# nkwangyh/CubemapSLAM

Hardware: AMD Instinct MI355X
Metric: frames/sec (extract+match+localBA) on Lafida cam0 (higher is better)
Workload: dtype u8 (extract/match), f64 (BA)

## Files before the change

cubemapslam_amd/api.py:

```python
import time
import ctypes as C
import os
import numpy as np

_HERE = os.path.dirname(os.path.abspath(__file__))
LIB_PATH = os.environ.get("CMS_HIP_LIB") or os.path.join(_HERE, "lib", "libcubemapslam_hip.so")


class CmsError(RuntimeError):
    pass


class Camera(C.Structure):
    _fields_ = [("c", C.c_double), ("d", C.c_double), ("e", C.c_double), ("u0", C.c_double), ("v0", C.c_double),
                ("invpol", C.c_double * 12), ("pol", C.c_double * 5), ("Iw", C.c_int), ("Ih", C.c_int),
                ("face", C.c_int), ("fov_deg", C.c_double)]


class OrbParams(C.Structure):
    _fields_ = [("nfeatures", C.c_int), ("scale_factor", C.c_float), ("nlevels", C.c_int),
                ("ini_th_fast", C.c_int), ("min_th_fast", C.c_int)]


class Geometry(C.Structure):
# ... 302 lines not shown
        f = lib().cms_stream_wait_extracted
        f.argtypes = [C.c_void_p, C.c_void_p]
        _chk(f(self.h, C.c_void_p(int(hip_stream))), "cms_stream_wait_extracted")

    def upload_wait(self):
        _chk(lib().cms_frames_upload_wait(self.h), "cms_frames_upload_wait")

    def process(self, B, from_fisheye=True):
        _chk(lib().cms_frames_process(self.h, B, 1 if from_fisheye else 0), "cms_frames_process")

    def sync(self):
        _chk(lib().cms_frames_sync(self.h), "cms_frames_sync")

    def fetch(self, b):
        cap = self.geom.kp_cap
        kps = np.zeros(cap, KP_DTYPE)
        desc = np.zeros((cap, 32), np.uint8)
        n = C.c_int()
        _chk(lib().cms_frames_fetch(self.h, b, _p(kps), _p(desc), cap, C.byref(n)), "cms_frames_fetch")
        return kps[:n.value].copy(), desc[:n.value].copy()

    def results_ptrs(self):
        a, b, c = C.c_void_p(), C.c_void_p(), C.c_void_p()
        _chk(lib().cms_frames_results(self.h, C.byref(a), C.byref(b), C.byref(c)), "cms_frames_results")
        return a.value, b.value, c.value

    def input_ptr(self):
        return lib().cms_frames_input(self.h)

    def profile(self, on=True):
        lib().cms_profile_enable(self.h, 1 if on else 0)

    def profile_ms(self):
        ms = np.zeros(7, np.float32)
        _chk(lib().cms_profile_get(self.h, _p(ms)), "cms_profile_get")
        return dict(zip(("remap", "pyramid", "fast", "octree", "cull", "describe", "total"), ms.tolist()))

    def debug_lut(self):
        W = self.W
        out = np.zeros((W, (W + 3) // 4 * 4), np.uint32)
        s = C.c_int()
        _chk(lib().cms_debug_lut(self.h, _p(out), C.byref(s)), "cms_debug_lut")
        return out[:, :W]

    def debug_level(self, b, l):
        w, h = self.geom.level_w[l], self.geom.level_h[l]
        out = np.zeros((h, w), np.uint8)
        _chk(lib().cms_debug_level(self.h, b, l, _p(out), w), "cms_debug_level")
        return out

    def debug_candidates(self, b, l):
        cap = self.geom.level_w[l] * self.geom.level_h[l] // 4 + 4096
        out = np.zeros((cap, 3), np.int32)
        n = C.c_int()
        _chk(lib().cms_debug_candidates(self.h, b, l, _p(out), cap, C.byref(n)), "cms_debug_candidates")
        return out[:n.value].copy()

    def debug_distributed(self, b, l):
        cap = self.geom.level_quota[l] + 8
        out = np.zeros((cap, 3), np.int32)
        n = C.c_int()
        _chk(lib().cms_debug_distributed(self.h, b, l, _p(out), cap, C.byref(n)), "cms_debug_distributed")
        return out[:n.value].copy()

    def hamming_best2(self, qdesc, tdesc, cand_off, cand_idx, tlevel=None, texcl=None):
        qdesc = np.ascontiguousarray(qdesc, np.uint8); tdesc = np.ascontiguousarray(tdesc, np.uint8)
        cand_off = np.ascontiguousarray(cand_off, np.int32); cand_idx = np.ascontiguousarray(cand_idx, np.int32)
        tl = np.ascontiguousarray(tlevel, np.int32) if tlevel is not None else None
        tx = np.ascontiguousarray(texcl, np.uint8) if texcl is not None else None
        nq = len(qdesc)
        outs = [np.zeros(max(nq, 1), np.int32) for _ in range(5)]
        _chk(lib().cms_hamming_best2(self.h, _p(qdesc), nq, _p(tdesc), len(tdesc), _p(cand_off), _p(cand_idx), _p(tl), _p(tx),
                                     *[_p(o) for o in outs]), "cms_hamming_best2")
        keys = ("best_idx", "best_dist", "best_level", "second_dist", "second_level")
        return {k: o[:nq] for k, o in zip(keys, outs)}

    def area_set_keypoints(self, b, kps):
        kps = np.ascontiguousarray(kps, KP_DTYPE)
        _chk(lib().cms_area_set_keypoints(self.h, b, len(kps), _p(kps)), "cms_area_set_keypoints")

    def area_grid(self, B):
        _chk(lib().cms_area_grid(self.h, B), "cms_area_grid")

    def features_in_area(self, b, qx, qy, qr, qmin, qmax, cap=None):
        qx = np.ascontiguousarray(qx, np.float32); qy = np.ascontiguousarray(qy, np.float32); qr = np.ascontiguousarray(qr, np.float32)
        qmin = np.ascontiguousarray(qmin, np.int32); qmax = np.ascontiguousarray(qmax, np.int32)
        nq = len(qx)
        cap = cap or max(1, 64 * nq + 1024)
        off = np.zeros(nq + 1, np.int32); idx = np.zeros(cap, np.int32); tot = C.c_int(0)
        _chk(lib().cms_features_in_area(self.h, b, nq, _p(qx), _p(qy), _p(qr), _p(qmin), _p(qmax), _p(off), _p(idx), cap, C.byref(tot)),
             "cms_features_in_area")
        return off, idx[:tot.value]

    def features_in_area_device(self, b, nq, d_q5, d_cnt, d_off, d_idx, cap, idx_base, d_total):
        _chk(lib().cms_features_in_area_device(self.h, b, nq, *[C.c_void_p(int(a)) for a in d_q5], C.c_void_p(int(d_cnt)), C.c_void_p(int(d_off)),
                                               C.c_void_p(int(d_idx)), cap, idx_base, C.c_void_p(int(d_total))), "cms_features_in_area_device")

    def features_in_area_batch_device(self, nq, d_qframe, d_q5, d_cnt, d_off, d_idx, cap, d_total):
        _chk(lib().cms_features_in_area_batch_device(self.h, nq, C.c_void_p(int(d_qframe)), *[C.c_void_p(int(a)) for a in d_q5], C.c_void_p(int(d_cnt)),
                                                     C.c_void_p(int(d_off)), C.c_void_p(int(d_idx)), cap, C.c_void_p(int(d_total))),
             "cms_features_in_area_batch_device")

    def area_set_descriptors(self, b, desc):
        desc = np.ascontiguousarray(desc, np.uint8)
        _chk(lib().cms_area_set_descriptors(self.h, b, len(desc), _p(desc)), "cms_area_set_descriptors")

    def search_local_points(self, b, pose15, pos, normal, min_dist, max_dist, mp_desc, kp_mp, viewing_cos_limit=0.5, th=1.0, nnratio=0.8,
                            th_high=100):
        pose15 = np.ascontiguousarray(pose15, np.float32).reshape(15)
        pos = np.ascontiguousarray(pos, np.float32).reshape(-1, 3); normal = np.ascontiguousarray(normal, np.float32).reshape(-1, 3)
        n = len(pos)
        min_dist = np.ascontiguousarray(min_dist, np.float32); max_dist = np.ascontiguousarray(max_dist, np.float32)
        mp_desc = np.ascontiguousarray(mp_desc, np.uint8).reshape(n, 32)
        assert kp_mp.dtype == np.int32 and kp_mp.flags.c_contiguous
        vis = np.zeros(n, np.uint8); px = np.zeros(n, np.float32); py = np.zeros(n, np.float32); lvl = np.zeros(n, np.int32)
        vc = np.zeros(n, np.float32); match = np.full(n, -1, np.int32)
        nm = C.c_int(0); rounds = C.c_int(0)
        _chk(lib().cms_search_local_points(self.h, b, _p(pose15), n, _p(pos), _p(normal), _p(min_dist), _p(max_dist), _p(mp_desc),
                                           viewing_cos_limit, th, nnratio, th_high, len(kp_mp), _p(kp_mp), _p(vis), _p(px), _p(py), _p(lvl),
                                           _p(vc), _p(match), C.addressof(nm), C.addressof(rounds)), "cms_search_local_points")
        return dict(in_view=vis, proj_x=px, proj_y=py, level=lvl, view_cos=vc, match=match, n_matches=nm.value, rounds=rounds.value)

    def search_local_points_ids(self, b, pose15, mpstore, ids, kp_mp, viewing_cos_limit=0.5, th=1.0, nnratio=0.8, th_high=100):
        pose15 = np.ascontiguousarray(pose15, np.float32).reshape(15)
        ids = _ids32(ids)
        n = len(ids)
        assert kp_mp.dtype == np.int32 and kp_mp.flags.c_contiguous
        vis = np.zeros(n, np.uint8); px = np.zeros(n, np.float32); py = np.zeros(n, np.float32); lvl = np.zeros(n, np.int32)
        vc = np.zeros(n, np.float32); match = np.full(n, -1, np.int32)
        nm = C.c_int(0); rounds = C.c_int(0)
        _chk(lib().cms_search_local_points_ids(self.h, b, _p(pose15), mpstore.h, n, _p(ids) if n else None, viewing_cos_limit, th, nnratio, th_high, len(kp_mp), _p(kp_mp),
                                               _p(vis), _p(px), _p(py), _p(lvl), _p(vc), _p(match), C.addressof(nm), C.addressof(rounds)), "cms_search_local_points_ids")
        return dict(in_view=vis, proj_x=px, proj_y=py, level=lvl, view_cos=vc, match=match, n_matches=nm.value, rounds=rounds.value)

    def search_by_projection(self, b, pose12, valid, Xw, octave, angle, mp_desc, kp_mp, th=15.0, check_ori=True, th_high=100):
        a = [np.ascontiguousarray(pose12, np.float32), np.ascontiguousarray(valid, np.uint8), np.ascontiguousarray(Xw, np.float32),
             np.ascontiguousarray(octave, np.int32), np.ascontiguousarray(angle, np.float32), np.ascontiguousarray(mp_desc, np.uint8)]
        n = len(a[1])
        match = np.full(n, -1, np.int32); nm = C.c_int(0)
        assert kp_mp.dtype == np.int32
        _chk(lib().cms_search_by_projection(self.h, b, _p(a[0]), n, *[_p(v) for v in a[1:]], th, int(check_ori), th_high, len(kp_mp), _p(kp_mp), _p(match),
                                            C.addressof(nm)), "cms_search_by_projection")
        return match, nm.value

    def search_by_projection_keyframe(self, b, pose12, kf_angle, pos, min_dist, max_dist, mp_desc, kp_mp, th=10.0, orb_dist=100, check_ori=True):
        a = [np.ascontiguousarray(pose12, np.float32).reshape(12), np.ascontiguousarray(kf_angle, np.float32), np.ascontiguousarray(pos, np.float32).reshape(-1, 3),
             np.ascontiguousarray(min_dist, np.float32), np.ascontiguousarray(max_dist, np.float32), np.ascontiguousarray(mp_desc, np.uint8).reshape(-1, 32)]
        n = len(a[1])
        assert all(len(v) == n for v in a[2:])
        assert kp_mp.dtype == np.int32 and kp_mp.flags.c_contiguous
        match = np.full(max(n, 1), -1, np.int32); nm = C.c_int(0)
        L = lib()
        L.cms_search_by_projection_keyframe.argtypes = ([C.c_void_p, C.c_int, C.c_void_p, C.c_int] + [C.c_void_p] * 5 + [C.c_float, C.c_int, C.c_int, C.c_int] +
                                                        [C.c_void_p] * 3)
        _chk(L.cms_search_by_projection_keyframe(self.h, b, _p(a[0]), n, *[_p(v) for v in a[1:]], float(th), int(orb_dist), int(check_ori), len(kp_mp), _p(kp_mp),
                                                 _p(match), C.addressof(nm)), "cms_search_by_projection_keyframe")
        return match[:n], nm.value

    def search_for_initialization(self, b2, k1, d1, prev_matched, window=100, nnratio=0.9, check_ori=True):
        k1 = np.ascontiguousarray(k1, KP_DTYPE); d1 = np.ascontiguousarray(d1, np.uint8)
        assert prev_matched.dtype == np.float32 and prev_matched.flags.c_contiguous and prev_matched.shape == (len(k1), 2)
        m12 = np.full(max(len(k1), 1), -1, np.int32); nm = C.c_int(0)
        f = lib().cms_search_for_initialization
        f.argtypes = [C.c_void_p, C.c_int, C.c_int, C.c_void_p, C.c_void_p, C.c_void_p, C.c_int, C.c_float, C.c_int, C.c_void_p, C.c_void_p]
        _chk(f(self.h, b2, len(k1), _p(k1), _p(d1), _p(prev_matched), int(window), float(nnratio), int(check_ori), _p(m12), C.addressof(nm)),
             "cms_search_for_initialization")
# ... 239 lines not shown
        L_.cms_vocab_transform.argtypes = [C.c_void_p, C.c_void_p, C.c_int, C.c_void_p, C.c_int] + [C.c_void_p] * 7
        self._create(device, int(k), int(L), int(scoring), int(weighting), len(parent), _p(parent), _p(is_leaf), _p(desc), _p(weight))

    @classmethod
    def from_dict(cls, t, device=0):
        return cls(t["k"], t["L"], t["scoring"], t["weighting"], t["parent"], t["is_leaf"], t["desc"], t["weight"], device=device)

    @classmethod
    def from_text_file(cls, path, device=0):
        return cls.from_dict(load_vocabulary_text(path), device=device)

    def info(self):
        a = np.zeros(7, np.int32)
        _chk(lib().cms_vocab_info(self.h, _p(a)), "cms_vocab_info")
        return dict(zip(("k", "L", "scoring", "weighting", "nodes", "words", "device"), (int(v) for v in a)))

    def transform(self, ctx, desc, levelsup=4):
        desc = np.ascontiguousarray(desc, np.uint8).reshape(-1, 32)
        n = len(desc)
        o = _bow_arrays(max(n, 1), max(n, 1), n)
        nw, nn = C.c_int(), C.c_int()
        _chk(lib().cms_vocab_transform(self.h, ctx.h, n, _p(desc) if n else None, int(levelsup), C.byref(nw), _p(o["word_id"]), _p(o["word_val"]), C.byref(nn),
                                       _p(o["node_id"]), _p(o["node_off"]), _p(o["node_feat"])), "cms_vocab_transform")
        return _bow_trim(o, nw.value, nn.value)


class KeyframeStore(_Handle):
    _entries = ("cms_kfstore_create", "cms_kfstore_destroy")

    def __init__(self, ctx, max_keyframes, max_features=2048, max_nodes=2048):
        self.ctx = ctx
        self.max_keyframes = int(max_keyframes)
        self._create(ctx.h, max_keyframes, max_features, max_nodes)

    def put(self, slot, K):
        _chk(lib().cms_kfstore_put(self.h, slot, C.byref(K)), "cms_kfstore_put")

    def update(self, slot, R=None, t=None, Ow=None, median_depth=None, mp=None):
        f = lambda a, dt: None if a is None else np.ascontiguousarray(a, dt)
        a = [f(R, np.float32), f(t, np.float32), f(Ow, np.float32), None if median_depth is None else np.array([median_depth], np.float32), f(mp, np.int32)]
        _chk(lib().cms_kfstore_update(self.h, slot, *[_p(v) for v in a]), "cms_kfstore_update")

    def put_from_frame(self, slot, src_ctx, b, n, kf):
        f32 = lambda a: np.ascontiguousarray(a, np.float32)
        i32 = lambda a: None if a is None else np.ascontiguousarray(a, np.int32)
        R, t, Ow = f32(np.asarray(kf["R"]).reshape(9)), f32(kf["t"]), f32(kf["Ow"])
        mp, nid, noff, nfeat = i32(kf.get("mp")), i32(kf["node_id"]), i32(kf["node_off"]), i32(kf["node_feat"])
        L = lib()
        _chk(L.cms_kfstore_put_from_frame(self.h, slot, src_ctx.h, b, n, _p(R), _p(t), _p(Ow), float(kf["median_depth"]), _p(mp), len(nid), _p(nid), _p(noff), _p(nfeat)),
             "cms_kfstore_put_from_frame")

    def put_from_frames(self, src_ctx, items):
        class KfFromFrame(C.Structure):
            _fields_ = [("slot", C.c_int), ("b", C.c_int), ("n", C.c_int), ("Rcw", C.c_void_p), ("tcw", C.c_void_p), ("Ow", C.c_void_p), ("median_depth", C.c_float),
                        ("mp", C.c_void_p), ("nnodes", C.c_int), ("node_id", C.c_void_p), ("node_off", C.c_void_p), ("node_feat", C.c_void_p)]
        arr = (KfFromFrame * len(items))()
        keep = []
        f32 = lambda a: np.ascontiguousarray(a, np.float32)
        i32 = lambda a: None if a is None else np.ascontiguousarray(a, np.int32)
        ptr = lambda a: None if a is None else a.ctypes.data
        for q, (slot, b, n, kf) in zip(arr, items):
            R, t, Ow = f32(np.asarray(kf["R"]).reshape(9)), f32(kf["t"]), f32(kf["Ow"])
            mp, nid, noff, nfeat = i32(kf.get("mp")), i32(kf["node_id"]), i32(kf["node_off"]), i32(kf["node_feat"])
            keep.append((R, t, Ow, mp, nid, noff, nfeat))
            q.slot = slot; q.b = b; q.n = n; q.Rcw = ptr(R); q.tcw = ptr(t); q.Ow = ptr(Ow); q.median_depth = float(kf["median_depth"]); q.mp = ptr(mp)
            q.nnodes = len(nid); q.node_id = ptr(nid); q.node_off = ptr(noff); q.node_feat = ptr(nfeat)
        L = lib()
        L.cms_kfstore_put_from_frames.argtypes = [C.c_void_p, C.c_void_p, C.c_int, C.c_void_p]
        _chk(L.cms_kfstore_put_from_frames(self.h, src_ctx.h, len(items), arr), "cms_kfstore_put_from_frames")

    def debug_fetch(self, slot, max_features=16384, max_nodes=16384):
        hdr = np.zeros(21, np.uint32); misc = np.zeros(2, np.int32)
        L = lib()
        _chk(L.cms_kfstore_debug_fetch(self.h, slot, *([None] * 10), _p(hdr), _p(misc)), "cms_kfstore_debug_fetch")
        n, nn = int(hdr[1]), int(hdr[3])
        o = dict(kps=np.zeros(n, KP_DTYPE), desc=np.zeros((n, 32), np.uint8), rays=np.zeros((n, 3), np.float32), mp=np.zeros(n, np.int32), feat_node=np.zeros(n, np.int32),
                 sorted=np.zeros(n, np.uint16), node_id=np.zeros(nn, np.int32), node_off=np.zeros(nn + 1, np.int32), node_feat=np.zeros(max(n, 1), np.int32),
                 cell_start=np.zeros(5 * 50 * 50 + 1, np.int32))
        _chk(L.cms_kfstore_debug_fetch(self.h, slot, _p(o["kps"]), _p(o["desc"]), _p(o["rays"]), _p(o["mp"]), _p(o["feat_node"]), _p(o["sorted"]), _p(o["node_id"]),
                                       _p(o["node_off"]), _p(o["node_feat"]), _p(o["cell_start"]), _p(hdr), _p(misc)), "cms_kfstore_debug_fetch")
        o["node_feat"] = o["node_feat"][:int(o["node_off"][-1]) if nn else 0]
        o["header"] = hdr; o["nvalid"] = int(misc[0]); o["kp_cnt"] = int(misc[1])
        return o

    def update_map_points(self, slot, feat, mp):
        a = [np.ascontiguousarray(v, np.int32).reshape(-1) for v in (slot, feat, mp)]
        assert len(a[0]) == len(a[1]) == len(a[2])
        L = lib()
        L.cms_kfstore_update_map_points.argtypes = [C.c_void_p, C.c_int] + [C.c_void_p] * 3
        pp = lambda v: _p(v) if len(v) else None
        _chk(L.cms_kfstore_update_map_points(self.h, len(a[0]), pp(a[0]), pp(a[1]), pp(a[2])), "cms_kfstore_update_map_points")

    def update_poses(self, slots, R, t, Ow):
        slots = np.ascontiguousarray(slots, np.int32)
        a = [np.ascontiguousarray(R, np.float32).reshape(-1), np.ascontiguousarray(t, np.float32).reshape(-1), np.ascontiguousarray(Ow, np.float32).reshape(-1)]
        assert len(a[0]) == 9 * len(slots) and len(a[1]) == 3 * len(slots) and len(a[2]) == 3 * len(slots)
        _chk(lib().cms_kfstore_update_poses(self.h, len(slots), _p(slots), _p(a[0]), _p(a[1]), _p(a[2])), "cms_kfstore_update_poses")

    def fuse_search(self, jobs, th=3.0):
        nj = len(jobs)
        slots = np.array([j[0] for j in jobs], np.int32)
        off = np.concatenate([[0], np.cumsum([len(j[1]["pos"]) for j in jobs])]).astype(np.int32)
        cat = lambda k, dt: np.ascontiguousarray(np.concatenate([np.asarray(j[1][k]) for j in jobs]), dt)
        a = [cat("skip", np.uint8), cat("pos", np.float32), cat("normal", np.float32), cat("min_dist", np.float32), cat("max_dist", np.float32), cat("desc", np.uint8)]
        n = int(off[-1])
        bi = np.zeros(n, np.int32); bd = np.zeros(n, np.int32)
        _chk(lib().cms_kfstore_fuse_search(self.h, nj, _p(slots), _p(off), *[_p(v) for v in a], th, _p(bi), _p(bd)), "cms_kfstore_fuse_search")
        return [(bi[off[j]:off[j + 1]].copy(), bd[off[j]:off[j + 1]].copy()) for j in range(nj)]

    def fuse_search_sets(self, sets, jobs, th=3.0):
        soff = np.concatenate([[0], np.cumsum([len(q["pos"]) for q in sets])]).astype(np.int32)
        cat = lambda k, dt: np.ascontiguousarray(np.concatenate([np.asarray(q[k]) for q in sets]), dt)
        a = [cat("pos", np.float32), cat("normal", np.float32), cat("min_dist", np.float32), cat("max_dist", np.float32), cat("desc", np.uint8)]
        slots = np.array([j[0] for j in jobs], np.int32); jset = np.array([j[1] for j in jobs], np.int32)
        sizes = [int(soff[j[1] + 1] - soff[j[1]]) for j in jobs]
        eoff = np.concatenate([[0], np.cumsum(sizes)]).astype(np.int64)
        skip = np.ascontiguousarray(np.concatenate([np.zeros(sz, np.uint8) if j[2] is None else np.asarray(j[2], np.uint8) for j, sz in zip(jobs, sizes)]), np.uint8)
        bi = np.zeros(int(eoff[-1]), np.int32); bd = np.zeros(int(eoff[-1]), np.int32)
        _chk(lib().cms_kfstore_fuse_search_sets(self.h, len(sets), _p(soff), *[_p(v) for v in a], len(jobs), _p(slots), _p(jset), _p(skip), th, _p(bi), _p(bd)),
             "cms_kfstore_fuse_search_sets")
        return [(bi[eoff[j]:eoff[j + 1]].copy(), bd[eoff[j]:eoff[j + 1]].copy()) for j in range(len(jobs))]

    def fuse_search_sets_ids(self, mpstore, sets, jobs, th=3.0):
        soff = np.concatenate([[0], np.cumsum([len(q) for q in sets])]).astype(np.int32)
        ids = _ids32(np.concatenate([np.asarray(q, np.int64).reshape(-1) for q in sets]) if len(sets) else [])
        slots = np.array([j[0] for j in jobs], np.int32); jset = np.array([j[1] for j in jobs], np.int32)
        sizes = [int(soff[j[1] + 1] - soff[j[1]]) for j in jobs]
        eoff = np.concatenate([[0], np.cumsum(sizes)]).astype(np.int64)
        skip = np.ascontiguousarray(np.concatenate([np.zeros(sz, np.uint8) if j[2] is None else np.asarray(j[2], np.uint8) for j, sz in zip(jobs, sizes)]), np.uint8)
        bi = np.zeros(max(int(eoff[-1]), 1), np.int32); bd = np.zeros(max(int(eoff[-1]), 1), np.int32)
        _chk(lib().cms_kfstore_fuse_search_sets_ids(self.h, mpstore.h, len(sets), _p(soff), _p(ids) if len(ids) else None, len(jobs), _p(slots), _p(jset), _p(skip), th,
                                                    _p(bi), _p(bd)), "cms_kfstore_fuse_search_sets_ids")
        return [(bi[eoff[j]:eoff[j + 1]].copy(), bd[eoff[j]:eoff[j + 1]].copy()) for j in range(len(jobs))]

    def create_new_map_points(self, jobs, check_orientation=False, cap=2048, copy=True):
        nj = len(jobs)
        key = (cap, tuple((int(j[0]), tuple(int(s) for s in j[1])) for j in jobs))
        st = getattr(self, "_cnmp", None)
        if st is None or st[0] != key:
            cur = np.array([j[0] for j in jobs], np.int32)
            neigh = np.array([s for j in jobs for s in j[1]] + [0], np.int32)
            off = np.concatenate([[0], np.cumsum([len(j[1]) for j in jobs])]).astype(np.int32)
            n_new = np.zeros(max(nj, 1), np.int32)
            on = np.zeros((max(nj, 1), cap), np.int32); o1 = np.zeros_like(on); o2 = np.zeros_like(on); ox = np.zeros((max(nj, 1), cap, 3), np.float32)
            arrs = (cur, off, neigh, n_new, on, o1, o2, ox)
            st = self._cnmp = (key, arrs, [_p(a) for a in arrs])
        cur, off, neigh, n_new, on, o1, o2, ox = st[1]
        pc, po, pn, pnn, pon, po1, po2, pox = st[2]
        t0 = time.perf_counter()
        _chk(lib().cms_kfstore_create_new_map_points(self.h, nj, pc, po, pn, int(check_orientation), cap, pnn, pon, po1, po2, pox), "cms_kfstore_create_new_map_points")
        self.last_call_ms = 1e3 * (time.perf_counter() - t0)
        if not copy:
            return [(on[j, :n_new[j]], o1[j, :n_new[j]], o2[j, :n_new[j]], ox[j, :n_new[j]]) for j in range(nj)]
        return [(on[j, :n_new[j]].copy(), o1[j, :n_new[j]].copy(), o2[j, :n_new[j]].copy(), ox[j, :n_new[j]].copy()) for j in range(nj)]

    def search_by_bow(self, src_ctx, jobs, nnratio=0.7, check_orientation=True):
        arr = (BowJob * max(len(jobs), 1))()
        keep = []
        for q, (slot, b, n, fv, skip) in zip(arr, jobs):
            nid, noff, nfeat = _bow_fv(fv)
            sk = None if skip is None else np.ascontiguousarray(skip, np.uint8)
            keep.append((nid, noff, nfeat, sk))
            q.slot = slot; q.b = b; q.n = n; q.nnodes = len(nid)
            q.node_id = nid.ctypes.data; q.node_off = noff.ctypes.data; q.node_feat = nfeat.ctypes.data; q.kf_skip = None if sk is None else sk.ctypes.data
        off = np.concatenate([[0], np.cumsum([int(j[2]) for j in jobs])]).astype(np.int64)
        kf_idx = np.full(max(int(off[-1]), 1), -1, np.int32); nm = np.zeros(max(len(jobs), 1), np.int32)
# ... 1115 lines not shown
```

cubemapslam_amd/csrc/cms_api_area.hip:

```cpp
#include <vector>

static int cms_area_grid_attr(int device) {
  static bool done[64] = {false};
  return cms_lds_ceiling_once((const void*)k_area_grid, (CMS_AREA_MAXKP + 1) * 8, device, done);
}
static int cms_area_reserve(cms_ctx* c) {
  if (c->d_area_sorted) return CMS_OK;
  if (c->g.kp_cap > CMS_AREA_MAXKP) return cms_fail(CMS_ERR_UNSUPPORTED, "frame grid: more than 16383 key points per frame");
  { const int rca = cms_area_grid_attr(c->device); if (rca) return rca; }
  const size_t B = (size_t)c->max_batch;
  HIPCHK(hipMalloc((void**)&c->d_area_sorted, B * c->g.kp_cap * sizeof(uint16_t)));
  HIPCHK(hipMalloc((void**)&c->d_area_cell_start, B * (CMS_AREA_CELLS + 1) * sizeof(int)));
  HIPCHK(hipMalloc((void**)&c->d_area_nvalid, B * sizeof(int)));
  return CMS_OK;
}

static int cms_area_tmp_reserve(cms_ctx* c, int nq) {
  if ((size_t)nq <= c->area_tmp_cap) return CMS_OK;
  if (c->d_area_tmp) hipFree(c->d_area_tmp);
  c->d_area_tmp = nullptr; c->area_tmp_cap = 0;
  const size_t cap = (size_t)nq + (size_t)nq / 4 + 1024;
  HIPCHK(hipMalloc((void**)&c->d_area_tmp, cap * CMS_AREA_TMP * sizeof(int)));
  c->area_tmp_cap = cap;
  return CMS_OK;
}
static int cms_area_psum_reserve(cms_ctx* c, int nparts) {
  if (nparts <= c->area_psum_cap) return CMS_OK;
  if (c->d_area_psum) hipFree(c->d_area_psum);
  c->d_area_psum = nullptr; c->area_psum_cap = 0;
  const int cap = nparts + nparts / 4 + 64;
  HIPCHK(hipMalloc((void**)&c->d_area_psum, (size_t)cap * sizeof(int)));
  c->area_psum_cap = cap;
  return CMS_OK;
}

static CmsAreaArgs cms_area_args(const CmsKeyPoint* kp, const uint16_t* sorted_idx, const int* cell_start, int kp_cap, int F, float inv) {
  CmsAreaArgs a = {};
  a.kp = kp; a.sorted_idx = sorted_idx; a.cell_start = cell_start; a.kp_cap = kp_cap; a.F = F; a.inv = inv;
  return a;
}
static CmsAreaArgs cms_area_args_frames(const cms_ctx* c, int b) {
  return cms_area_args((const CmsKeyPoint*)c->d_kps + (size_t)b * c->g.kp_cap, c->d_area_sorted + (size_t)b * c->g.kp_cap,
                       c->d_area_cell_start + (size_t)b * (CMS_AREA_CELLS + 1), c->g.kp_cap, c->g.F, cms_grid_inv(c));
}
static void cms_area_queries(CmsAreaArgs& a, int nq, const void* q_frame, const void* qx, const void* qy, const void* qr, const void* qmin, const void* qmax,
                             void* cnt, void* off, void* idx, int cap, int idx_base) {
  a.nq = nq; a.q_frame = (const int*)q_frame;
  a.qx = (const float*)qx; a.qy = (const float*)qy; a.qr = (const float*)qr; a.qmin = (const int*)qmin; a.qmax = (const int*)qmax;
  a.cnt = (int*)cnt; a.off = (int*)off; a.idx = (int*)idx; a.cap = cap; a.idx_base = idx_base;
}
struct CmsWindowCols {
  size_t o0 = 0, stride = 0;
  float *qx, *qy, *qr; int *qmin, *qmax, *level, *slot, *rec, *cnt, *off, *idx;
  void take(CmsBlock& b, size_t E) {
    o0 = b.size; stride = cms_align(E * 4);
    for (int k = 0; k < 9; ++k) b.take(E * 4);
    b.take(E * 4, 4);
  }
  void at(uint8_t* p, size_t o_idx) {
    float* f = (float*)(p + o0); int* i = (int*)(p + o0);
    const size_t n = stride / 4;
    qx = f; qy = f + n; qr = f + 2 * n; qmin = i + 3 * n; qmax = i + 4 * n; level = i + 5 * n; slot = i + 6 * n; rec = i + 7 * n; cnt = i + 8 * n; off = i + 9 * n;
    idx = (int*)(p + o_idx);
  }
};
static void cms_area_queries(CmsAreaArgs& a, int nq, const CmsWindowCols& w, int cap) {
  cms_area_queries(a, nq, w.slot, w.qx, w.qy, w.qr, w.qmin, w.qmax, w.cnt, w.off, w.idx, cap, 0);
}
static int cms_area_launch(cms_ctx* c, hipStream_t s, CmsAreaArgs a, void* d_total) {
  const int nq = a.nq, qgrid = cms_area_search_grid(nq);
  int rc = cms_area_psum_reserve(c, qgrid);
  if (rc) return rc;
  rc = cms_area_tmp_reserve(c, nq);
  if (rc) return rc;
  a.tmp = c->d_area_tmp; a.psum = c->d_area_psum;
  hipLaunchKernelGGL(k_area_query, dim3(qgrid), dim3(CMS_AREA_QT), 0, s, a);
  hipLaunchKernelGGL(k_area_lists, dim3(cms_area_tile_grid(nq)), dim3(CMS_AREA_LT), 0, s, a, (int*)d_total);
  HIPCHK(hipGetLastError());
  return CMS_OK;
}

extern "C" int cms_area_set_keypoints(cms_ctx* c, int b, int n, const cms_keypoint* kps) {
  if (!c || b < 0 || b >= c->max_batch || n < 0 || n > c->g.kp_cap || (n > 0 && !kps)) return cms_fail(CMS_ERR_ARG, "cms_area_set_keypoints: bad argument");
  HIPCHK(hipSetDevice(c->device));
  if (n > 0) HIPCHK(hipMemcpyAsync(c->d_kps + (size_t)b * c->g.kp_cap, kps, (size_t)n * sizeof(cms_keypoint), hipMemcpyHostToDevice, c->stream));
  HIPCHK(hipMemcpyAsync(c->d_kp_cnt + b, &n, sizeof(int), hipMemcpyHostToDevice, c->stream));
  HIPCHK(hipStreamSynchronize(c->stream));
  return CMS_OK;
}

extern "C" int cms_area_grid(cms_ctx* c, int B) {
  if (!c || B < 1 || B > c->max_batch) return cms_fail(CMS_ERR_ARG, "cms_area_grid: bad batch");
  HIPCHK(hipSetDevice(c->device));
  int rc = cms_area_reserve(c);
  if (rc) return rc;
  hipLaunchKernelGGL(k_area_grid, dim3(B), dim3(1024), (size_t)(c->g.kp_cap + 1) * 8, c->stream, (const CmsKeyPoint*)c->d_kps, (const int*)c->d_kp_cnt, c->g.kp_cap, c->g.F, cms_grid_inv(c),
                     c->d_area_sorted, c->d_area_cell_start, c->d_area_nvalid);
  HIPCHK(hipGetLastError());
  c->area_frames = B;
  return CMS_OK;
}

extern "C" int cms_features_in_area_device(cms_ctx* c, int b, int nq, const void* d_qx, const void* d_qy, const void* d_qr, const void* d_qmin,
                                           const void* d_qmax, void* d_cnt_scratch, void* d_cand_off, void* d_cand_idx, int cap, int idx_base,
                                           void* d_total) {
  if (!c || b < 0 || b >= c->area_frames || nq < 0 || cap < 0) return cms_fail(CMS_ERR_ARG, "cms_features_in_area_device: bad argument (cms_area_grid first)");
  if (nq == 0) return CMS_OK;
  HIPCHK(hipSetDevice(c->device));
  CmsAreaArgs a = cms_area_args_frames(c, b);
  cms_area_queries(a, nq, nullptr, d_qx, d_qy, d_qr, d_qmin, d_qmax, d_cnt_scratch, d_cand_off, d_cand_idx, cap, idx_base);
  return cms_area_launch(c, c->stream, a, d_total);
}

extern "C" int cms_features_in_area_batch_device(cms_ctx* c, int nq, const void* d_qframe, const void* d_qx, const void* d_qy, const void* d_qr,
                                                 const void* d_qmin, const void* d_qmax, void* d_cnt_scratch, void* d_cand_off, void* d_cand_idx,
                                                 int cap, void* d_total) {
  if (!c || nq < 0 || cap < 0 || c->area_frames < 1 || !d_qframe) return cms_fail(CMS_ERR_ARG, "cms_features_in_area_batch_device: bad argument (cms_area_grid first)");
  if (nq == 0) return CMS_OK;
  HIPCHK(hipSetDevice(c->device));
  CmsAreaArgs a = cms_area_args_frames(c, 0);
  cms_area_queries(a, nq, d_qframe, d_qx, d_qy, d_qr, d_qmin, d_qmax, d_cnt_scratch, d_cand_off, d_cand_idx, cap, 0);
  return cms_area_launch(c, c->stream, a, d_total);
}

extern "C" int cms_features_in_area(cms_ctx* c, int b, int nq, const float* qx, const float* qy, const float* qr, const int* qmin, const int* qmax,
                                    int* cand_off, int* cand_idx, int cap, int* total) {
  if (!c || nq < 0 || cap < 0 || !cand_off || (nq > 0 && (!qx || !qy || !qr || !qmin || !qmax))) return cms_fail(CMS_ERR_ARG, "cms_features_in_area: bad argument");
  if (b < 0 || b >= c->area_frames) return cms_fail(CMS_ERR_ARG, "cms_features_in_area: no grid for this frame (cms_area_grid first)");
  cand_off[0] = 0;
  if (total) *total = 0;
  if (nq == 0) return CMS_OK;
  HIPCHK(hipSetDevice(c->device));
  const size_t qb = (size_t)nq * 4;
  const size_t bytes = 5 * qb + qb  + (qb + 4)  + (size_t)cap * 4 + 64;
  hipStream_t s = c->stream;
  int rc = c->stage.reserve(s, bytes, 0);
  if (rc) return rc;
  uint8_t* p = c->stage.d;
  void* dq[5];
  const void* hq[5] = {qx, qy, qr, qmin, qmax};
  for (int i = 0; i < 5; ++i) { dq[i] = p; p += qb; HIPCHK(hipMemcpyAsync(dq[i], hq[i], qb, hipMemcpyHostToDevice, s)); }
  void* d_cnt = p; p += qb;
  void* d_off = p; p += qb + 4;
  void* d_tot = p; p += 16;
  void* d_idx = p;
  rc = cms_features_in_area_device(c, b, nq, dq[0], dq[1], dq[2], dq[3], dq[4], d_cnt, d_off, d_idx, cap, 0, d_tot);
  if (rc) return rc;
  int tot = 0;
  HIPCHK(hipMemcpyAsync(cand_off, d_off, qb + 4, hipMemcpyDeviceToHost, s));
  HIPCHK(hipMemcpyAsync(&tot, d_tot, sizeof(int), hipMemcpyDeviceToHost, s));
  HIPCHK(hipStreamSynchronize(s));
  if (total) *total = tot;
  if (tot > cap) return cms_fail(CMS_ERR_OVERFLOW, "cms_features_in_area: candidate capacity too small");
  if (tot > 0 && cand_idx) HIPCHK(hipMemcpy(cand_idx, d_idx, (size_t)tot * 4, hipMemcpyDeviceToHost));
  return CMS_OK;
}
```

cubemapslam_amd/csrc/cms_api_frames.hip:

```cpp
#include <chrono>
#include <thread>
#include <hip/hip_runtime.h>
#include <math.h>
#include <stdio.h>
#include <stdlib.h>
#include <string.h>
#include <algorithm>
#include <string>
#include <vector>
#include "../../include/cubemapslam_hip.h"
#include "cms_types.h"
#include "cms_stage.h"
#include "orb_pattern.inc"

static bool cms_cu_mask_from_env(uint32_t* words, int* n_words) {
  const char* v = getenv("CMS_CTX_CU_MASK");
  if (!v || !*v) return false;
  int n = 0;
  while (*v && n < 8) {
    char* end = nullptr;
    words[n++] = (uint32_t)strtoul(v, &end, 16);
    if (end == v) return false;
    v = *end == ',' ? end + 1 : end;
    if (*end && *end != ',') return false;
  }
  *n_words = n;
  return n > 0;
}

struct CmsCtxBow;
static void cms_ctx_bow_free(CmsCtxBow* b);
static void cms_ctx_bow_invalidate(CmsCtxBow* b);

struct CmsHipMem;
using CmsStage = CmsStageT<CmsHipMem>;

static thread_local std::string g_cms_err;
static int cms_fail(int code, const char* what, hipError_t e = hipSuccess) {
  char buf[512];
  if (e != hipSuccess) snprintf(buf, sizeof(buf), "%s: %s", what, hipGetErrorString(e));
  else snprintf(buf, sizeof(buf), "%s", what);
  g_cms_err = buf;
  return code;
}
#define HIPCHK(call)                                                        \
  do {                                                                      \
    hipError_t _e = (call);                                                 \
    if (_e != hipSuccess) return cms_fail(CMS_ERR_HIP, #call, _e);          \
  } while (0)

extern "C" const char* cms_last_error(void) { return g_cms_err.c_str(); }
extern "C" int cms_device_count(void) {
  int n = 0;
  if (hipGetDeviceCount(&n) != hipSuccess) return 0;
  return n;
}

struct cms_ctx {
  int device = 0;
  cms_camera cam;
  cms_orb_params orb;
  int max_batch = 0;
  CmsGeom g;
  float scale[CMS_MAX_LEVELS], inv_scale[CMS_MAX_LEVELS], sigma2[CMS_MAX_LEVELS], inv_sigma2[CMS_MAX_LEVELS];
  hipStream_t stream = nullptr;
  int fstride = 0;
  size_t fish_pitch = 0;
  int lut_stride = 0, mstride = 0;
  bool have_mask = false;
  int dirty_frames = 0;
  uint8_t* d_fish = nullptr; uint32_t* d_lut = nullptr; uint8_t* d_pyr = nullptr; uint8_t* d_mask = nullptr;
  cms_remap_tile* d_rtiles = nullptr; int rt_mode = 1, rt_tw = 64, rt_live = 0, rt_all = 0, rt_lds = 0;
  CmsResizeTab* d_tab = nullptr; float* d_pattern = nullptr;
  uint32_t* d_cand = nullptr; uint16_t* d_node = nullptr; int* d_cand_cnt = nullptr; int* d_overflow = nullptr;
  uint32_t* d_qt_out = nullptr; int* d_qt_cnt = nullptr;
  uint32_t* d_cell_cand = nullptr; int* d_cell_cnt = nullptr;
  int* d_cells_all = nullptr; int* d_cells_live = nullptr; int n_cells_all = 0, n_cells_live = 0;
  uint16_t* d_area_sorted = nullptr; int* d_area_cell_start = nullptr; int* d_area_nvalid = nullptr; int area_frames = 0;
  int* d_area_psum = nullptr; int area_psum_cap = 0;
  int* d_area_tmp = nullptr; size_t area_tmp_cap = 0;
  uint8_t* h_fish_stage = nullptr; int fish_stage_frames = 0;
  hipStream_t copy_stream = nullptr; hipEvent_t ev_upload_done = nullptr, ev_remap_done = nullptr;
  bool upload_pending = false, remap_recorded = false;
  int dist_bounds_scaled = 0;
  hipEvent_t ev_block = nullptr; int last_batch = 0;
  hipEvent_t ev_extracted = nullptr; bool extracted_recorded = false;
  CmsKeyPoint* d_kps = nullptr; uint32_t* d_aux = nullptr; uint8_t* d_desc = nullptr; int* d_kp_cnt = nullptr;
  uint32_t* d_order = nullptr; uint32_t* d_aux_sorted = nullptr; int* d_walk_cnt = nullptr; float* d_rays = nullptr;
  CmsStage stage;
  bool prof = false;
  bool desc_spatial = false;
  hipEvent_t ev[8] = {nullptr, nullptr, nullptr, nullptr, nullptr, nullptr, nullptr, nullptr};
  size_t fast_lds = 0, qt_lds = 0;
  CmsCtxBow* bow = nullptr;
};

static inline double cms_horner12(const double* c, double x) {
  double r = 0.0;
  for (int i = 11; i >= 0; --i) r = r * x + c[i];
  return r;
}
static void cms_cubemap_to_fisheye(const cms_camera& cam, double up, double vp, double* uf, double* vf) {
  const int F = cam.face;
  const double half = F / 2.0;
  float i = (float)up, j = (float)vp;
  *uf = -1; *vf = -1;
  const float fi = i / (float)F, fj = j / (float)F;
  int face = CMS_FACE_UNKNOWN;
  if (fi >= 0 && fi < 1 && fj >= 1 && fj < 2) face = CMS_FACE_LEFT;
  else if (fi >= 1 && fi < 2 && fj >= 0 && fj < 1) face = CMS_FACE_UPPER;
  else if (fi >= 1 && fi < 2 && fj >= 1 && fj < 2) face = CMS_FACE_FRONT;
  else if (fi >= 1 && fi < 2 && fj >= 2 && fj < 3) face = CMS_FACE_LOWER;
  else if (fi >= 2 && fi < 3 && fj >= 1 && fj < 2) face = CMS_FACE_RIGHT;
  if (face == CMS_FACE_UNKNOWN) return;
  i = i - (float)((int)(i / (float)F) * F);
  j = j - (float)((int)(j / (float)F) * F);
  const double lx = ((double)i - half) * 1.0 / half, ly = ((double)j - half) * 1.0 / half, lz = 1.0;
  double x, y, z;
  switch (face) {
    case CMS_FACE_FRONT: x = lx; y = ly; z = lz; break;
    case CMS_FACE_LEFT: x = -lz; y = ly; z = lx; break;
    case CMS_FACE_RIGHT: x = lz; y = ly; z = -lx; break;
    case CMS_FACE_LOWER: x = lx; y = lz; z = -ly; break;
    default: x = lx; y = -lz; z = ly; break;
  }
  double norm = sqrt(x * x + y * y);
  if (norm == 0.0) norm = 1e-14;
  const double theta = atan(-z / norm);
  const double rho = cms_horner12(cam.invpol, theta);
  const double uu = x / norm * rho, vv = y / norm * rho;
  *uf = uu * cam.c + vv * cam.d + cam.u0;
  *vf = uu * cam.e + vv + cam.v0;
  if (*uf < 0 || *uf >= cam.Iw || *vf < 0 || *vf >= cam.Ih) { *uf = -1; *vf = -1; }
}
static void cms_build_lut(const cms_camera& cam, int lut_stride, std::vector<uint32_t>& lut) {
  const int W = 3 * cam.face;
  lut.assign((size_t)W * lut_stride, 0u);
  for (int y = 0; y < W; ++y)
    for (int x = 0; x < W; ++x) {
      double u, v;
      cms_cubemap_to_fisheye(cam, (double)x, (double)y, &u, &v);
      if (u < 0 || v < 0 || u >= cam.Iw || v >= cam.Ih) continue;
      const float mu = (float)u, mv = (float)v;
      const int sx = (int)lrint((double)(mu * 32.f)), sy = (int)lrint((double)(mv * 32.f));
      const uint32_t X = (uint32_t)(sx >> 5), Y = (uint32_t)(sy >> 5), ax = (uint32_t)(sx & 31), ay = (uint32_t)(sy & 31);
      lut[(size_t)y * lut_stride + x] = X | (Y << 11) | (ax << 22) | (ay << 27);
    }
}

extern "C" int cms_remap_lut_host(const cms_camera* cam, uint32_t* lut, int lut_stride) {
  if (!cam || !lut || cam->face < 1 || lut_stride < 3 * cam->face) return cms_fail(CMS_ERR_ARG, "cms_remap_lut_host: bad argument");
  std::vector<uint32_t> v;
  cms_build_lut(*cam, lut_stride, v);
  memcpy(lut, v.data(), v.size() * 4);
  return CMS_OK;
}
extern "C" int cms_remap_tiles_host(const cms_camera* cam, const uint32_t* lut, int lut_stride, int tile_w, int tile_h, int lds_budget,
                                    cms_remap_tile* out, int cap, int* n_live, int* n_all, int* lds_bytes) {
  if (!cam || !lut || !out || !n_live || !n_all || !lds_bytes || cam->face < 1 || lut_stride < 3 * cam->face || !cms_rt_shape_ok(tile_w, tile_h) || lds_budget < 0)
    return cms_fail(CMS_ERR_ARG, "cms_remap_tiles_host: bad argument");
  std::vector<cms_remap_tile> v;
// ... 110 lines not shown
          const bool corner = !(y >= F && y < 2 * F) && (x < F || x >= 2 * F);
          cls[(size_t)y * lv.w + x] = corner ? CMS_CLS_ZERO : lut[(size_t)y * lut_stride + x] == 0 ? CMS_CLS_PIX00 : CMS_CLS_VARYING;
        }
    } else {
      const CmsLevel& sv = g.lv[l - 1];
      const CmsResizeTab* tx = &tab[lv.tab_off];
      const CmsResizeTab* ty = tx + lv.w;
      std::vector<uint8_t> okx(lv.w), oky(lv.h);
      for (int x = 0; x < lv.w; ++x) okx[x] = (int)tx[x].a0 + (int)tx[x].a1 == 2048 && tx[x].a0 >= 0 && tx[x].a1 >= 0;
      for (int y = 0; y < lv.h; ++y) {
        const uint32_t b0 = (uint32_t)ty[y].a0 & 0xFFFu, b1 = (uint32_t)ty[y].a1 & 0xFFFu;
        bool ok = ty[y].a0 >= 0 && ty[y].a1 >= 0;
        for (uint32_t c = 0; c < 256 && ok; ++c) {
          const uint32_t h = ((c * 2048u) >> 4) & 0xFFFFu;
          ok = (int)(((b0 * h) >> 16) + ((b1 * h) >> 16) + 2) >> 2 == (int)c;
        }
        oky[y] = ok;
      }
      for (int y = 0; y < lv.h; ++y) {
        const int r0 = std::min(std::max((int)ty[y].s, 0), sv.h - 1), r1 = std::min(std::max((int)ty[y].s + 1, 0), sv.h - 1);
        for (int x = 0; x < lv.w; ++x) {
          const int c0 = tx[x].s, c1 = std::min((int)tx[x].s + 1, sv.w - 1);
          const uint8_t k = prev[(size_t)r0 * sv.w + c0];
          if (k != CMS_CLS_VARYING && okx[x] && oky[y] && prev[(size_t)r0 * sv.w + c1] == k && prev[(size_t)r1 * sv.w + c0] == k && prev[(size_t)r1 * sv.w + c1] == k)
            cls[(size_t)y * lv.w + x] = k;
        }
      }
    }
    const int maxBX = lv.w - CMS_MINB, maxBY = lv.h - CMS_MINB;
    for (int ci = 0; ci < lv.nRows; ++ci)
      for (int cj = 0; cj < lv.nCols; ++cj) {
        const int iniY = CMS_MINB + ci * lv.hCell, iniX = CMS_MINB + cj * lv.wCell;
        if (iniY >= maxBY - 3 || iniX >= maxBX - 6) continue;
        const int maxY = std::min(iniY + lv.hCell + 6, maxBY), maxX = std::min(iniX + lv.wCell + 6, maxBX);
        if (maxX - iniX - 6 <= 0 || maxY - iniY - 6 <= 0) continue;
        const int id = l | (ci << 4) | (cj << 12);
        all.push_back(id);
        const bool zero = (maxX <= lv.zlo || iniX >= lv.w - lv.zhi) && (maxY <= lv.zlo || iniY >= lv.h - lv.zhi);
        if (zero) continue;
        nz.push_back(id);
        const uint8_t k = cls[(size_t)iniY * lv.w + iniX];
        bool constant = k != CMS_CLS_VARYING;
        for (int y = iniY; y < maxY && constant; ++y)
          for (int x = iniX; x < maxX; ++x) if (cls[(size_t)y * lv.w + x] != k) { constant = false; break; }
        if (!constant) live.push_back(id);
      }
  }
  auto xcd_stripe = [](std::vector<int>& v) {
    if (getenv("CMS_FAST_NO_XCD_STRIPE")) return;
    const size_t n = v.size(), per = (n + 7) / 8;
    std::vector<int> out;
    out.reserve(n);
    for (size_t j = 0; j < per; ++j)
      for (size_t x = 0; x < 8; ++x) if (x * per + j < n) out.push_back(v[x * per + j]);
    v.swap(out);
  };
  xcd_stripe(all); xcd_stripe(nz); xcd_stripe(live);
  return CMS_OK;
}

extern "C" int cms_fast_cells_host(const cms_camera* cam, const cms_orb_params* orb, int which, int* out, int cap, int* n) {
  if (!cam || !orb || !n || which < 0 || which > 2 || cap < 0 || (cap > 0 && !out)) return cms_fail(CMS_ERR_ARG, "cms_fast_cells_host: bad argument");
  if (cam->Iw < 2 || cam->Ih < 2 || cam->Iw > 2047 || cam->Ih > 2047) return cms_fail(CMS_ERR_UNSUPPORTED, "fisheye size must be <= 2047");
  CmsGeom g;
  CmsLevelSetup ls{};
  { const int rc = cms_level_geometry(cam, orb, g, &ls); if (rc != CMS_OK) return rc; }
  const int lut_stride = (int)cms_align((size_t)g.W, 4);
  std::vector<uint32_t> lut;
  cms_build_lut(*cam, lut_stride, lut);
  std::vector<CmsResizeTab> tab;
  std::vector<int> lists[3];
  { const int rc = cms_fast_cell_lists(g, ls.tab_off, lut.data(), lut_stride, tab, lists[0], lists[1], lists[2]); if (rc != CMS_OK) return rc; }
  *n = (int)lists[which].size();
  if (*n > cap) return cap == 0 ? CMS_OK : cms_fail(CMS_ERR_OVERFLOW, "cms_fast_cells_host: caller capacity too small");
  if (*n) memcpy(out, lists[which].data(), (size_t)*n * sizeof(int));
  return CMS_OK;
}

static void cms_ctx_free(cms_ctx* c) {
  if (!c) return;
  hipSetDevice(c->device);
  void* ptrs[] = {c->d_fish, c->d_lut, c->d_pyr, c->d_mask, c->d_tab, c->d_pattern, c->d_cand, c->d_node, c->d_cand_cnt,
                  c->d_overflow, c->d_qt_out, c->d_qt_cnt, c->d_kps, c->d_aux, c->d_order, c->d_aux_sorted, c->d_desc, c->d_kp_cnt, c->d_cell_cand,
                  c->d_cell_cnt, c->d_cells_all, c->d_cells_live, c->d_area_sorted, c->d_area_cell_start, c->d_area_nvalid, c->d_area_psum, c->d_area_tmp, c->d_walk_cnt, c->d_rays, c->d_rtiles};
  for (void* p : ptrs) if (p) hipFree(p);
  cms_ctx_bow_free(c->bow);
  if (c->h_fish_stage) (void)hipHostFree(c->h_fish_stage);
  c->stage.release();
  for (int i = 0; i < 8; ++i) if (c->ev[i]) hipEventDestroy(c->ev[i]);
  if (c->ev_extracted) hipEventDestroy(c->ev_extracted);
  if (c->ev_block) hipEventDestroy(c->ev_block);
  if (c->ev_upload_done) hipEventDestroy(c->ev_upload_done);
  if (c->ev_remap_done) hipEventDestroy(c->ev_remap_done);
  if (c->copy_stream) hipStreamDestroy(c->copy_stream);
  if (c->stream) hipStreamDestroy(c->stream);
  delete c;
}

extern "C" int cms_ctx_create(cms_ctx** out, int device, const cms_camera* cam, const cms_orb_params* orb, int max_batch) {
  if (!out || !cam || !orb || max_batch < 1) return cms_fail(CMS_ERR_ARG, "cms_ctx_create: bad argument");
  *out = nullptr;
  if (orb->nlevels < 1 || orb->nlevels > CMS_MAX_LEVELS) return cms_fail(CMS_ERR_UNSUPPORTED, "nlevels must be 1..12");
  if (cam->face < 32 || 3 * cam->face > 4095) return cms_fail(CMS_ERR_UNSUPPORTED, "face size must satisfy 32 <= F and 3F <= 4095");
  if (cam->Iw < 2 || cam->Ih < 2 || cam->Iw > 2047 || cam->Ih > 2047) return cms_fail(CMS_ERR_UNSUPPORTED, "fisheye size must be <= 2047");
  int ndev = 0;
  if (hipGetDeviceCount(&ndev) != hipSuccess || ndev == 0) return cms_fail(CMS_ERR_NO_DEVICE, "no HIP device: the product path has no CPU fallback");
  if (device < 0 || device >= ndev) return cms_fail(CMS_ERR_ARG, "device index out of range");
  HIPCHK(hipSetDevice(device));
  cms_ctx* c = new cms_ctx;
  c->device = device; c->cam = *cam; c->orb = *orb; c->max_batch = max_batch;
  CmsGeom& g = c->g;
  const int L = orb->nlevels, F = cam->face, W = 3 * F;
  CmsLevelSetup ls{};
  { const int rc = cms_level_geometry(cam, orb, g, &ls); if (rc != CMS_OK) { delete c; return rc; } }
  memcpy(c->scale, ls.scale, sizeof(c->scale)); memcpy(c->inv_scale, ls.inv_scale, sizeof(c->inv_scale));
  memcpy(c->sigma2, ls.sigma2, sizeof(c->sigma2)); memcpy(c->inv_sigma2, ls.inv_sigma2, sizeof(c->inv_sigma2));
  const size_t tab_off = ls.tab_off;
  const int maxq = ls.maxq, wCellMax = ls.wCellMax, hCellMax = ls.hCellMax;
  g.qt_maxn = 8;
  while (g.qt_maxn < maxq + 3) g.qt_maxn <<= 1;
  if (g.qt_maxn > 2048) { delete c; return cms_fail(CMS_ERR_UNSUPPORTED, "per-level feature quota above 2045 is not supported"); }
  g.tile_h = hCellMax + 6;
  g.tile_stride = (int)cms_align((size_t)wCellMax + 6 + 3, 4) + 4;
  g.sc_h = hCellMax + 2;
  g.sc_stride = (int)cms_align((size_t)wCellMax + 2, 4);
  g.list_cap = wCellMax * hCellMax;
  g.cell_cap = (int)cms_align((size_t)((wCellMax + 1) / 2) * ((hCellMax + 1) / 2), 8);
  g.dbg_stop = getenv("CMS_DBG_FAST_STOP") ? atoi(getenv("CMS_DBG_FAST_STOP")) : 0;
  c->desc_spatial = getenv("CMS_DESC_SPATIAL_ORDER") != nullptr && g.kp_cap <= CMS_ORDER_MAX && max_batch <= 65535;
  g.gauss_column_mode = 0;
  if (wCellMax > 60 || hCellMax > 60) { delete c; return cms_fail(CMS_ERR_UNSUPPORTED, "FAST cell larger than 60 pixels"); }
  if (orb->scale_factor < 1.01f || orb->scale_factor > 1.9f) { delete c; return cms_fail(CMS_ERR_UNSUPPORTED, "scaleFactor must be in [1.01, 1.9]"); }
  g.fast_cell_lds = (int)cms_align((size_t)g.tile_h * g.tile_stride + (size_t)g.sc_h * g.sc_stride + 2 * (size_t)g.list_cap + 16, 16);
  c->fast_lds = CMS_FAST_WPB * (size_t)g.fast_cell_lds;
  c->qt_lds = 64 * (size_t)g.qt_maxn + 4 * 512 + 64;

  c->fstride = (int)cms_align((size_t)cam->Iw, 64);
  c->fish_pitch = (size_t)c->fstride * cam->Ih;
  c->lut_stride = (int)cms_align((size_t)W, 4);
  c->mstride = (int)cms_align((size_t)W, 64);
  const size_t B = (size_t)max_batch;
#define ALLOC(ptr, bytes) do { hipError_t _e = hipMalloc((void**)&(ptr), (bytes)); if (_e != hipSuccess) { cms_ctx_free(c); return cms_fail(CMS_ERR_HIP, "hipMalloc " #ptr, _e); } } while (0)
  hipError_t e;
  {
    const char* pr = getenv("CMS_FRAME_STREAM_PRIORITY");
    int lo = 0, hi = 0;
    uint32_t cu_mask[8]; int cu_words = 0;
    if (cms_cu_mask_from_env(cu_mask, &cu_words))
      e = hipExtStreamCreateWithCUMask(&c->stream, (uint32_t)cu_words, cu_mask);
    else
    if (pr && hipDeviceGetStreamPriorityRange(&lo, &hi) == hipSuccess && lo != hi)
      e = hipStreamCreateWithPriority(&c->stream, hipStreamNonBlocking, pr[0] == 'h' ? hi : lo);
    else
      e = hipStreamCreateWithFlags(&c->stream, hipStreamNonBlocking);
  }
  if (e != hipSuccess) { cms_ctx_free(c); return cms_fail(CMS_ERR_HIP, "hipStreamCreate", e); }
  for (int i = 0; i < 8; ++i) hipEventCreate(&c->ev[i]);
  ALLOC(c->d_fish, B * c->fish_pitch + 256);
  ALLOC(c->d_lut, (size_t)W * c->lut_stride * 4);
  ALLOC(c->d_pyr, B * g.pyr_bytes + 256);
  ALLOC(c->d_mask, (size_t)W * c->mstride);
  ALLOC(c->d_tab, tab_off * sizeof(CmsResizeTab));
  ALLOC(c->d_pattern, 1024 * sizeof(float));
  ALLOC(c->d_cand, B * g.cand_total * 4);
  ALLOC(c->d_node, B * g.cand_total * 2);
  ALLOC(c->d_cand_cnt, B * L * sizeof(int));
  ALLOC(c->d_overflow, sizeof(int));
// ... 541 lines not shown
```

cubemapslam_amd/csrc/cms_api_tri.hip:

```cpp
#include <algorithm>
#include <cmath>
#include <cstdlib>
#include <cstring>
#include <memory>
#include <mutex>
#include <vector>

namespace {
inline float tri_h_small(const float* a, const float* b, int bs) {
  float t = a[0] * b[0];
  t = t + a[1] * b[bs];
  t = t + a[2] * b[2 * bs];
  return t;
}
void tri_h_e12(const float* R1w, const float* t1w, const float* R2w, const float* t2w, float* E12) {
  float R12[9], M[9], t12[3];
  for (int r = 0; r < 3; ++r)
    for (int c = 0; c < 3; ++c) {
      double s = 0;
      for (int k = 0; k < 3; ++k) s += (double)R1w[3 * r + k] * (double)R2w[3 * c + k];
      R12[3 * r + c] = (float)(s * 1.0);
      M[3 * r + c] = (float)(s * -1.0);
    }
  for (int r = 0; r < 3; ++r) t12[r] = (float)((double)tri_h_small(M + 3 * r, t2w, 1) * 1.0 + (double)t1w[r] * 1.0);
// ... 206 lines not shown
  if (nneigh < 0 || (nneigh > 0 && !neigh)) return cms_fail(CMS_ERR_ARG, "cms_create_new_map_points: bad neighbour list");
  const int nkf = njobs + nneigh;
  std::vector<CmsTriKF> kfs;
  std::vector<float> median;
  auto kf_at = [&](int i) -> const cms_keyframe& { return i < njobs ? cur[i] : neigh[i - njobs]; };
  TriDev dev;
  size_t o_work = 0;
  int max_n1 = 1;
  int rc = tri_flatten_upload(c, nkf, kf_at, njobs, "cms_create_new_map_points: bad key frame (at most 4096 features)", kfs, median, dev, o_work, max_n1,
                              [&](int mn1) { return TriWork(njobs, nneigh, mn1, cap_per_job).bytes; });
  if (rc) return rc;
  uint8_t* p = c->stage.d;
  std::vector<int> cur_idx((size_t)njobs), neigh_idx((size_t)nneigh + 1);
  for (int j = 0; j < njobs; ++j) cur_idx[(size_t)j] = j;
  for (int q = 0; q < nneigh; ++q) neigh_idx[(size_t)q] = njobs + q;
  return tri_run(c, dev, kfs.data(), median.data(), njobs, cur_idx.data(), neigh_off, neigh_idx.data(), check_orientation, cap_per_job, p + o_work, n_new,
                 out_neigh, out_idx1, out_idx2, out_x3d);
}

extern "C" int cms_search_for_triangulation(cms_ctx* c, const cms_keyframe* kf1, const cms_keyframe* kf2, const float* E12, int check_orientation,
                                            int* matches12, int* n_matches) {
  if (!c || !kf1 || !kf2 || !matches12 || !n_matches) return cms_fail(CMS_ERR_ARG, "cms_search_for_triangulation: bad argument");
  if (c->g.nlevels > 16 || c->g.nlevels < 2) return cms_fail(CMS_ERR_UNSUPPORTED, "cms_search_for_triangulation: 2..16 pyramid levels");
  *n_matches = 0;
  if (kf1->n == 0) return CMS_OK;
  std::vector<CmsTriKF> kfs;
  std::vector<float> median;
  auto kf_at = [&](int i) -> const cms_keyframe& { return i == 0 ? *kf1 : *kf2; };
  TriDev dev;
  size_t o_work = 0;
  int max_n1 = 1;
  CmsBlock blk;
  const size_t o_pair = blk.take(sizeof(CmsTriPair), 16), o_job = blk.take(sizeof(CmsTriJob), 16), o_m = blk.size;
  int rc = tri_flatten_upload(c, 2, kf_at, 1, "cms_search_for_triangulation: bad key frame (at most 4096 features)", kfs, median, dev, o_work, max_n1,
                              [&](int mn1) { return o_m + cms_align((size_t)mn1 * 4 + 16) + 256; });
  if (rc) return rc;
  uint8_t* p = c->stage.d + o_work;
  const size_t o_n = o_m + cms_align((size_t)max_n1 * 4 + 16);
  CmsTriPair pr;
  pr.kf2 = 1; pr.skip = 0;
  if (E12) std::memcpy(pr.E12, E12, sizeof(pr.E12));
  else tri_h_e12(kfs[0].Rcw, kfs[0].tcw, kfs[1].Rcw, kfs[1].tcw, pr.E12);
  float C2[3];
  for (int r = 0; r < 3; ++r) C2[r] = (float)((double)tri_h_small(kfs[1].Rcw + 3 * r, kfs[0].Ow, 1) * 1.0 + (double)kfs[1].tcw[r] * 1.0);
  track_rays_to_cubemap(c->g.F, C2[0], C2[1], C2[2], pr.ex, pr.ey);
  CmsTriJob jb; jb.kf1 = 0; jb.pair0 = 0; jb.npairs = 1;
  hipStream_t s = c->stream;
  HIPCHK(hipMemcpyAsync(p + o_pair, &pr, sizeof(pr), hipMemcpyHostToDevice, s));
  HIPCHK(hipMemcpyAsync(p + o_job, &jb, sizeof(jb), hipMemcpyHostToDevice, s));
  CmsTriArgs a;
  std::memset(&a, 0, sizeof(a));
  a.kf = dev.kf; a.pair = (const CmsTriPair*)(p + o_pair); a.job = (const CmsTriJob*)(p + o_job);
  a.kp = dev.kp; a.desc = dev.desc; a.rays = dev.rays; a.mp = dev.mp; a.feat_node = dev.feat_node;
  a.node_id = dev.node_id; a.node_off = dev.node_off; a.node_feat = dev.node_feat;
  a.F = c->g.F;
  a.check_orientation = check_orientation;
  cms_level_table(a.sf, c, c->scale, 1.0f); cms_level_table(a.sigma2, c, c->sigma2, 1.0f);
  hipLaunchKernelGGL(k_tri_search, dim3(1), dim3(1024), 0, s, a, (int*)(p + o_m), (int*)(p + o_n));
  HIPCHK(hipGetLastError());
  HIPCHK(hipMemcpyAsync(matches12, p + o_m, (size_t)kf1->n * 4, hipMemcpyDeviceToHost, s));
  HIPCHK(hipMemcpyAsync(n_matches, p + o_n, 4, hipMemcpyDeviceToHost, s));
  HIPCHK(hipStreamSynchronize(s));
  return CMS_OK;
}

struct CmsStoreBow;
static void cms_store_bow_free(CmsStoreBow* b);
static void cms_store_bow_invalidate(CmsStoreBow* b, int slot);
struct CmsStoreKfdb;
static CmsStoreKfdb* cms_store_kfdb_new(int max_keyframes);
static void cms_store_kfdb_free(CmsStoreKfdb* d);
static void cms_store_kfdb_refill(CmsStoreKfdb* d, int slot);
struct CmsStoreMpUpd;
static void cms_store_mpupd_free(CmsStoreMpUpd* u);
struct cms_kfstore {
  cms_ctx* c = nullptr;
  CmsStoreBow* bow = nullptr;
  CmsStoreKfdb* kfdb = nullptr;
  CmsStoreMpUpd* mpupd = nullptr;
  int maxkf = 0, maxf = 0, maxn = 0;
  CmsTriKF* d_kf = nullptr; CmsKeyPoint* d_kp = nullptr; uint8_t* d_desc = nullptr; float* d_rays = nullptr; int* d_mp = nullptr; int* d_fn = nullptr;
  int* d_nid = nullptr; int* d_noff = nullptr; int* d_nfeat = nullptr;
  uint8_t* d_work = nullptr; size_t work_bytes = 0;
  uint16_t* d_sorted = nullptr; int* d_cell_start = nullptr; int* d_nvalid = nullptr; int* d_kp_cnt = nullptr;
  std::vector<CmsTriKF> h_kf; std::vector<float> h_median; std::vector<uint8_t> used;
  struct PutCall { hipEvent_t ev = nullptr; ~PutCall() { if (ev) (void)hipEventDestroy(ev); } };
  int* h_ff = nullptr; size_t ff_stride = 0; std::vector<std::shared_ptr<PutCall>> ff_call;
  void* h_items = nullptr; int items_gen = 0; std::shared_ptr<PutCall> items_call[2];
  unsigned upd_call = 0; hipEvent_t upd_ev[4] = {nullptr, nullptr, nullptr, nullptr}; bool upd_ev_set[4] = {false, false, false, false};
  std::vector<uint8_t> busy; hipEvent_t order_ev = nullptr;
  std::mutex put_mu; std::vector<std::shared_ptr<PutCall>> pending_puts;
  float* h_upd = nullptr; std::vector<uint8_t> upd_par;
};

static hipError_t kfstore_order_behind_puts(cms_kfstore* st);
template <class SlotOfJob>
static int kfstore_wait_puts(const cms_kfstore* st, hipStream_t stream, int njobs, SlotOfJob&& slot_of_job) {
  for (int j = 0; j < njobs; ++j) {
    const auto& call = st->ff_call[(size_t)slot_of_job(j)];
    if (call) HIPCHK(hipStreamWaitEvent(stream, call->ev, 0));
  }
  return CMS_OK;
}
extern "C" void cms_kfstore_destroy(cms_kfstore* st) {
  if (!st) return;
  if (st->c) (void)hipSetDevice(st->c->device);
  void* bufs[] = {st->d_kf, st->d_kp, st->d_desc, st->d_rays, st->d_mp, st->d_fn, st->d_nid, st->d_noff, st->d_nfeat, st->d_work,
                  st->d_sorted, st->d_cell_start, st->d_nvalid, st->d_kp_cnt};
  for (void* b : bufs) if (b) (void)hipFree(b);
  cms_store_bow_free(st->bow);
  cms_store_kfdb_free(st->kfdb);
  cms_store_mpupd_free(st->mpupd);
  if (st->h_ff) (void)hipHostFree(st->h_ff);
  if (st->h_items) (void)hipHostFree(st->h_items);
  if (st->h_upd) (void)hipHostFree(st->h_upd);
  for (hipEvent_t e : st->upd_ev) if (e) (void)hipEventDestroy(e);
  if (st->order_ev) (void)hipEventDestroy(st->order_ev);
  delete st;
}

extern "C" int cms_kfstore_create(cms_kfstore** out, cms_ctx* c, int max_keyframes, int max_features, int max_nodes) {
  if (!out || !c || max_keyframes < 1 || max_features < 1 || max_features > CMS_AREA_MAXKP || max_nodes < 1)
    return cms_fail(CMS_ERR_ARG, "cms_kfstore_create: bad argument (at most 16383 features per key frame)");
  HIPCHK(hipSetDevice(c->device));
  { const int rca = cms_area_grid_attr(c->device); if (rca) return rca; }
  cms_kfstore* st = new cms_kfstore();
  st->c = c; st->maxkf = max_keyframes; st->maxf = max_features; st->maxn = max_nodes;
  const size_t K = (size_t)max_keyframes, Fq = (size_t)max_features, Nq = (size_t)max_nodes;
#define KF_ALLOC(ptr, bytes) do { if (hipMalloc((void**)&(ptr), (bytes)) != hipSuccess) { cms_kfstore_destroy(st); return cms_fail(CMS_ERR_HIP, "cms_kfstore_create: out of device memory"); } } while (0)
  KF_ALLOC(st->d_kf, K * sizeof(CmsTriKF));
  KF_ALLOC(st->d_kp, K * Fq * sizeof(CmsKeyPoint));
  KF_ALLOC(st->d_desc, K * Fq * 32);
  KF_ALLOC(st->d_rays, K * Fq * 12);
  KF_ALLOC(st->d_mp, K * Fq * 4);
  KF_ALLOC(st->d_fn, K * Fq * 4);
  KF_ALLOC(st->d_nid, K * Nq * 4);
  KF_ALLOC(st->d_noff, K * (Nq + 1) * 4);
  KF_ALLOC(st->d_nfeat, K * Fq * 4);
  KF_ALLOC(st->d_sorted, K * Fq * sizeof(uint16_t));
  KF_ALLOC(st->d_cell_start, K * (CMS_AREA_CELLS + 1) * sizeof(int));
  KF_ALLOC(st->d_nvalid, K * sizeof(int));
  KF_ALLOC(st->d_kp_cnt, K * sizeof(int));
#undef KF_ALLOC
  st->kfdb = cms_store_kfdb_new(max_keyframes);
  if (!st->kfdb) { cms_kfstore_destroy(st); return cms_fail(CMS_ERR_HIP, "cms_kfstore_create: out of device memory"); }
  st->h_kf.assign(K, CmsTriKF{}); st->h_median.assign(K, 1.0f); st->used.assign(K, 0); st->busy.assign(K, 0);
  st->ff_call.assign(K, nullptr);
  *out = st;
  return CMS_OK;
}

extern "C" int cms_kfstore_put(cms_kfstore* st, int slot, const cms_keyframe* kf) {
  if (!st || !kf || slot < 0 || slot >= st->maxkf) return cms_fail(CMS_ERR_ARG, "cms_kfstore_put: bad argument");
  int rc = tri_check_keyframe(*kf, "cms_kfstore_put: bad key frame");
  if (rc) return rc;
  if (kf->n > st->maxf || kf->nnodes > st->maxn) return cms_fail(CMS_ERR_ARG, "cms_kfstore_put: key frame larger than the store's slots");
  cms_ctx* c = st->c;
  HIPCHK(hipSetDevice(c->device));
  HIPCHK(kfstore_order_behind_puts(st));
  hipStream_t s = c->stream;
  const size_t f0 = (size_t)slot * st->maxf, n0 = (size_t)slot * st->maxn, o0 = (size_t)slot * (st->maxn + 1);
  CmsTriKF d;
  d.f0 = (int)f0; d.n = kf->n; d.node0 = (int)n0; d.nnodes = kf->nnodes; d.noff0 = (int)o0; d.nfeat0 = (int)f0;
  std::memcpy(d.Rcw, kf->Rcw, sizeof(d.Rcw)); std::memcpy(d.tcw, kf->tcw, sizeof(d.tcw)); std::memcpy(d.Ow, kf->Ow, sizeof(d.Ow));
  std::vector<int> fn((size_t)kf->n + 1, -1);
  tri_feat_node(*kf, fn.data());
  const int zero = 0;
  if (kf->n > 0) {
    HIPCHK(hipMemcpyAsync(st->d_kp + f0, kf->kps, (size_t)kf->n * sizeof(CmsKeyPoint), hipMemcpyHostToDevice, s));
    HIPCHK(hipMemcpyAsync(st->d_desc + 32 * f0, kf->desc, 32 * (size_t)kf->n, hipMemcpyHostToDevice, s));
    HIPCHK(hipMemcpyAsync(st->d_rays + 3 * f0, kf->rays, 12 * (size_t)kf->n, hipMemcpyHostToDevice, s));
    HIPCHK(hipMemcpyAsync(st->d_mp + f0, kf->mp, 4 * (size_t)kf->n, hipMemcpyHostToDevice, s));
    HIPCHK(hipMemcpyAsync(st->d_fn + f0, fn.data(), 4 * (size_t)kf->n, hipMemcpyHostToDevice, s));
  }
  if (kf->nnodes > 0) {
    HIPCHK(hipMemcpyAsync(st->d_nid + n0, kf->node_id, 4 * (size_t)kf->nnodes, hipMemcpyHostToDevice, s));
    HIPCHK(hipMemcpyAsync(st->d_noff + o0, kf->node_off, 4 * ((size_t)kf->nnodes + 1), hipMemcpyHostToDevice, s));
    if (kf->node_off[kf->nnodes] > 0) HIPCHK(hipMemcpyAsync(st->d_nfeat + f0, kf->node_feat, 4 * (size_t)kf->node_off[kf->nnodes], hipMemcpyHostToDevice, s));
  } else {
    HIPCHK(hipMemcpyAsync(st->d_noff + o0, &zero, 4, hipMemcpyHostToDevice, s));
  }
  HIPCHK(hipMemcpyAsync(st->d_kf + slot, &d, sizeof(d), hipMemcpyHostToDevice, s));
  HIPCHK(hipMemcpyAsync(st->d_kp_cnt + slot, &kf->n, sizeof(int), hipMemcpyHostToDevice, s));
  hipLaunchKernelGGL(k_area_grid, dim3(1), dim3(1024), (size_t)(st->maxf + 1) * 8, s, (const CmsKeyPoint*)(st->d_kp + f0), (const int*)(st->d_kp_cnt + slot), st->maxf, c->g.F,
                     cms_grid_inv(c), st->d_sorted + f0, st->d_cell_start + (size_t)slot * (CMS_AREA_CELLS + 1), st->d_nvalid + slot);
  HIPCHK(hipGetLastError());
  HIPCHK(hipStreamSynchronize(s));
  st->h_kf[(size_t)slot] = d; st->h_median[(size_t)slot] = kf->median_depth; st->used[(size_t)slot] = 1;
  cms_store_bow_invalidate(st->bow, slot);
  cms_store_kfdb_refill(st->kfdb, slot);
  return CMS_OK;
}

struct CmsKfFromFrame {
  const CmsKeyPoint* kp; const uint8_t* desc; const float* rays; const uint16_t* sorted; const int* cell_start; const int* nvalid;
  CmsKeyPoint* o_kp; uint8_t* o_desc; float* o_rays; uint16_t* o_sorted; int* o_cell_start; int* o_nvalid; int* o_kp_cnt;
  int* o_mp; int* o_fn; int* o_nid; int* o_noff; int* o_nfeat; CmsTriKF* o_kf;
  const int* h_mp; const int* h_fn; const int* h_nid; const int* h_noff; const int* h_nfeat;
  CmsTriKF kf; int n, nnodes, nfeat;
};
extern "C" __global__ void __launch_bounds__(256) k_kf_put_from_frame(const CmsKfFromFrame* __restrict__ items) {
  const CmsKfFromFrame a = items[blockIdx.y];
  const int gs = gridDim.x * blockDim.x, t0 = blockIdx.x * blockDim.x + threadIdx.x;
  const int n = a.n;
  {
    const uint32_t* s = reinterpret_cast<const uint32_t*>(a.kp); uint32_t* d = reinterpret_cast<uint32_t*>(a.o_kp);
    for (int i = t0; i < 6 * n; i += gs) d[i] = s[i];
  }
  {
    const uint4* s = reinterpret_cast<const uint4*>(a.desc); uint4* d = reinterpret_cast<uint4*>(a.o_desc);
    for (int i = t0; i < 2 * n; i += gs) d[i] = s[i];
  }
  for (int i = t0; i < 3 * n; i += gs) a.o_rays[i] = a.rays[i];
  for (int i = t0; i < n; i += gs) { a.o_sorted[i] = a.sorted[i]; a.o_mp[i] = a.h_mp ? a.h_mp[i] : -1; a.o_fn[i] = a.h_fn[i]; }
  for (int i = t0; i <= CMS_AREA_CELLS; i += gs) a.o_cell_start[i] = a.cell_start[i];
  for (int i = t0; i < a.nnodes; i += gs) a.o_nid[i] = a.h_nid[i];
  for (int i = t0; i <= a.nnodes; i += gs) a.o_noff[i] = a.nnodes > 0 ? a.h_noff[i] : 0;
  for (int i = t0; i < a.nfeat; i += gs) a.o_nfeat[i] = a.h_nfeat[i];
  if (t0 == 0) { *a.o_nvalid = *a.nvalid; *a.o_kp_cnt = n; *a.o_kf = a.kf; }
}
static hipError_t kfstore_order_behind_puts(cms_kfstore* st) {
  std::vector<std::shared_ptr<cms_kfstore::PutCall>> w;
  { std::lock_guard<std::mutex> lk(st->put_mu); w.swap(st->pending_puts); }
  for (auto& c : w) { const hipError_t e = hipStreamWaitEvent(st->c->stream, c->ev, 0); if (e != hipSuccess) return e; }
  return hipSuccess;
}
static int kfstore_ff_reserve(cms_kfstore* st) {
  if (st->h_ff) return CMS_OK;
  st->ff_stride = ((size_t)3 * st->maxf + 2 * (size_t)st->maxn + 1 + 63) & ~(size_t)63;
  HIPCHK(hipHostMalloc((void**)&st->h_ff, (size_t)st->maxkf * st->ff_stride * sizeof(int), hipHostMallocMapped | hipHostMallocCoherent));
  HIPCHK(hipHostMalloc((void**)&st->h_items, 2 * (size_t)st->maxkf * sizeof(CmsKfFromFrame), hipHostMallocMapped | hipHostMallocCoherent));
  return CMS_OK;
}
static int kf_put_check(cms_kfstore* st, int slot, cms_ctx* src, int b, int n, const float* Rcw, const float* tcw, const float* Ow,
                        const int* mp, int nnodes, const int* node_id, const int* node_off, const int* node_feat) {
  if (slot < 0 || slot >= st->maxkf || b < 0 || b >= src->max_batch || n < 0 || nnodes < 0 || !Rcw || !tcw || !Ow ||
      (nnodes > 0 && (!node_id || !node_off || !node_feat)))
    return cms_fail(CMS_ERR_ARG, "cms_kfstore_put_from_frame: bad argument");
  cms_ctx* c = st->c;
  if (b >= src->area_frames) return cms_fail(CMS_ERR_ARG, "cms_kfstore_put_from_frame: no frame grid for this frame (cms_area_grid on the batch first)");
  if (n > st->maxf || n > src->g.kp_cap || nnodes > st->maxn) return cms_fail(CMS_ERR_ARG, "cms_kfstore_put_from_frame: key frame larger than the store's slots");
  {
    cms_keyframe chk;
    std::memset(&chk, 0, sizeof(chk));
    chk.n = n; chk.nnodes = nnodes; chk.node_id = node_id; chk.node_off = node_off; chk.node_feat = node_feat;
    chk.kps = reinterpret_cast<const cms_keypoint*>(st); chk.desc = reinterpret_cast<const uint8_t*>(st); chk.rays = reinterpret_cast<const float*>(st); chk.mp = reinterpret_cast<const int*>(st);
    const int rc = tri_check_keyframe(chk, "cms_kfstore_put_from_frame: bad key frame");
    if (rc) return rc;
  }
  const int nfeat = nnodes > 0 ? node_off[nnodes] : 0;
  if (nfeat > st->maxf) return cms_fail(CMS_ERR_ARG, "cms_kfstore_put_from_frame: FeatureVector lists more features than the slot holds");
  (void)c; (void)mp;
  return CMS_OK;
}
static int kf_put_fill(cms_kfstore* st, int slot, cms_ctx* src, int b, int n, const float* Rcw, const float* tcw, const float* Ow,
                       const int* mp, int nnodes, const int* node_id, const int* node_off, const int* node_feat, CmsKfFromFrame& a) {
  const int nfeat = nnodes > 0 ? node_off[nnodes] : 0;
  if (st->ff_call[(size_t)slot]) { HIPCHK(hipEventSynchronize(st->ff_call[(size_t)slot]->ev)); st->ff_call[(size_t)slot].reset(); }
  int* h = st->h_ff + (size_t)slot * st->ff_stride;
  int* h_mp = h; int* h_fn = h + st->maxf; int* h_nfeat = h + 2 * (size_t)st->maxf; int* h_nid = h + 3 * (size_t)st->maxf; int* h_noff = h_nid + st->maxn;
  if (mp && n > 0) std::memcpy(h_mp, mp, 4 * (size_t)n);
  {
    static thread_local std::vector<int> fn;
    fn.assign((size_t)std::max(n, 1), -1);
    for (int e = 0; e < nnodes; ++e)
      for (int q = node_off[e]; q < node_off[e + 1]; ++q) fn[(size_t)node_feat[q]] = e;
    if (n > 0) std::memcpy(h_fn, fn.data(), 4 * (size_t)n);
  }
  if (nnodes > 0) { std::memcpy(h_nid, node_id, 4 * (size_t)nnodes); std::memcpy(h_noff, node_off, 4 * ((size_t)nnodes + 1)); std::memcpy(h_nfeat, node_feat, 4 * (size_t)nfeat); }
  const size_t f0 = (size_t)slot * st->maxf, n0 = (size_t)slot * st->maxn, o0 = (size_t)slot * (st->maxn + 1);
  std::memset(&a, 0, sizeof(a));
  CmsTriKF& d = a.kf;
  d.f0 = (int)f0; d.n = n; d.node0 = (int)n0; d.nnodes = nnodes; d.noff0 = (int)o0; d.nfeat0 = (int)f0;
  std::memcpy(d.Rcw, Rcw, sizeof(d.Rcw)); std::memcpy(d.tcw, tcw, sizeof(d.tcw)); std::memcpy(d.Ow, Ow, sizeof(d.Ow));
  const size_t sb = (size_t)b * src->g.kp_cap;
  a.kp = (const CmsKeyPoint*)src->d_kps + sb; a.desc = src->d_desc + 32 * sb; a.rays = src->d_rays + 3 * sb; a.sorted = src->d_area_sorted + sb;
  a.cell_start = src->d_area_cell_start + (size_t)b * (CMS_AREA_CELLS + 1); a.nvalid = src->d_area_nvalid + b;
  a.o_kp = st->d_kp + f0; a.o_desc = st->d_desc + 32 * f0; a.o_rays = st->d_rays + 3 * f0; a.o_sorted = st->d_sorted + f0;
  a.o_cell_start = st->d_cell_start + (size_t)slot * (CMS_AREA_CELLS + 1); a.o_nvalid = st->d_nvalid + slot; a.o_kp_cnt = st->d_kp_cnt + slot;
  a.o_mp = st->d_mp + f0; a.o_fn = st->d_fn + f0; a.o_nid = st->d_nid + n0; a.o_noff = st->d_noff + o0; a.o_nfeat = st->d_nfeat + f0; a.o_kf = st->d_kf + slot;
  a.h_mp = mp ? h_mp : nullptr; a.h_fn = h_fn; a.h_nid = h_nid; a.h_noff = h_noff; a.h_nfeat = h_nfeat;
  a.n = n; a.nnodes = nnodes; a.nfeat = nfeat;
  return CMS_OK;
}
extern "C" int cms_kfstore_put_from_frames(cms_kfstore* st, cms_ctx* src, int n_items, const cms_kf_from_frame* items) {
  if (!st || !src || n_items < 0 || n_items > st->maxkf || (n_items > 0 && !items)) return cms_fail(CMS_ERR_ARG, "cms_kfstore_put_from_frames: bad argument");
  if (n_items == 0) return CMS_OK;
  cms_ctx* c = st->c;
  if (src->device != c->device || src->g.F != c->g.F || src->g.W != c->g.W) return cms_fail(CMS_ERR_ARG, "cms_kfstore_put_from_frame: the frame context and the store must share device and cubemap geometry");
  HIPCHK(hipSetDevice(c->device));
  { const int rc = kfstore_ff_reserve(st); if (rc) return rc; }
  {
    std::vector<uint8_t> seen((size_t)st->maxkf, 0);
    for (int i = 0; i < n_items; ++i) {
      const cms_kf_from_frame& q = items[i];
      const int rc = kf_put_check(st, q.slot, src, q.b, q.n, q.Rcw, q.tcw, q.Ow, q.mp, q.nnodes, q.node_id, q.node_off, q.node_feat);
      if (rc) return rc;
      if (seen[(size_t)q.slot]) return cms_fail(CMS_ERR_ARG, "cms_kfstore_put_from_frames: a slot is named twice");
      seen[(size_t)q.slot] = 1;
    }
  }
  const int gen = (st->items_gen ^= 1);
  if (st->items_call[gen]) { HIPCHK(hipEventSynchronize(st->items_call[gen]->ev)); st->items_call[gen].reset(); }
  CmsKfFromFrame* h_items = reinterpret_cast<CmsKfFromFrame*>(st->h_items) + (size_t)gen * st->maxkf;
  int max_n = 0;
  for (int i = 0; i < n_items; ++i) {
    const cms_kf_from_frame& q = items[i];
    const int rc = kf_put_fill(st, q.slot, src, q.b, q.n, q.Rcw, q.tcw, q.Ow, q.mp, q.nnodes, q.node_id, q.node_off, q.node_feat, h_items[i]);
    if (rc) return rc;
    max_n = std::max(max_n, q.n);
  }
  hipStream_t s = src->stream;
  {
    bool wait = false;
    for (int i = 0; i < n_items; ++i) wait = wait || (st->busy[(size_t)items[i].slot] != 0);
    if (wait && c->stream != s) {
      if (!st->order_ev) HIPCHK(hipEventCreateWithFlags(&st->order_ev, hipEventDisableTiming));
      HIPCHK(hipEventRecord(st->order_ev, c->stream));
      HIPCHK(hipStreamWaitEvent(s, st->order_ev, 0));
      std::fill(st->busy.begin(), st->busy.end(), 0);
    }
  }
  hipLaunchKernelGGL(k_kf_put_from_frame, dim3(std::max(1, std::min(32, (6 * max_n + 255) / 256)), n_items), dim3(256), 0, s, (const CmsKfFromFrame*)h_items);
  HIPCHK(hipGetLastError());
  auto call = std::make_shared<cms_kfstore::PutCall>();
  HIPCHK(hipEventCreateWithFlags(&call->ev, hipEventDisableTiming));
  HIPCHK(hipEventRecord(call->ev, s));
  if (c->stream != s) { std::lock_guard<std::mutex> lk(st->put_mu); st->pending_puts.push_back(call); }
  for (int i = 0; i < n_items; ++i) {
    const cms_kf_from_frame& q = items[i];
    st->ff_call[(size_t)q.slot] = call;
    st->h_kf[(size_t)q.slot] = h_items[i].kf; st->h_median[(size_t)q.slot] = q.median_depth; st->used[(size_t)q.slot] = 1;
    cms_store_bow_invalidate(st->bow, q.slot);
    cms_store_kfdb_refill(st->kfdb, q.slot);
  }
  st->items_call[gen] = call;
  return CMS_OK;
}
extern "C" int cms_kfstore_put_from_frame(cms_kfstore* st, int slot, cms_ctx* src, int b, int n, const float* Rcw, const float* tcw, const float* Ow,
                                          float median_depth, const int* mp, int nnodes, const int* node_id, const int* node_off, const int* node_feat) {
  cms_kf_from_frame q;
  q.slot = slot; q.b = b; q.n = n; q.Rcw = Rcw; q.tcw = tcw; q.Ow = Ow; q.median_depth = median_depth; q.mp = mp; q.nnodes = nnodes;
  q.node_id = node_id; q.node_off = node_off; q.node_feat = node_feat;
  return cms_kfstore_put_from_frames(st, src, 1, &q);
}

extern "C" __global__ void __launch_bounds__(64) k_kf_update_poses(CmsTriKF* kf, const float* upd, const int* __restrict__ list, int n) {
  const int i = blockIdx.x * blockDim.x + threadIdx.x;
  if (i >= n) return;
  const int slot = list[i] & 0x3FFFFFFF, par = (list[i] >> 30) & 1;
  const float* u = upd + 16 * (2 * (size_t)slot + par);
  CmsTriKF& d = kf[slot];
  for (int j = 0; j < 9; ++j) d.Rcw[j] = u[j];
  for (int j = 0; j < 3; ++j) { d.tcw[j] = u[9 + j]; d.Ow[j] = u[12 + j]; }
}
extern "C" int cms_kfstore_update_poses(cms_kfstore* st, int n, const int* slots, const float* Rcw, const float* tcw, const float* Ow) {
  if (!st || n < 0 || n > st->maxkf || (n > 0 && (!slots || !Rcw || !tcw || !Ow))) return cms_fail(CMS_ERR_ARG, "cms_kfstore_update_poses: bad argument");
  for (int i = 0; i < n; ++i) if (slots[i] < 0 || slots[i] >= st->maxkf || !st->used[(size_t)slots[i]]) return cms_fail(CMS_ERR_ARG, "cms_kfstore_update_poses: bad slot");
  if (n == 0) return CMS_OK;
  cms_ctx* c = st->c;
  HIPCHK(hipSetDevice(c->device));
  HIPCHK(kfstore_order_behind_puts(st));
  if (!st->h_upd) {
    HIPCHK(hipHostMalloc((void**)&st->h_upd, (size_t)st->maxkf * (32 * sizeof(float) + 4 * sizeof(int)), hipHostMallocMapped | hipHostMallocCoherent));
    st->upd_par.assign((size_t)st->maxkf, 0);
  }
  const unsigned ring = st->upd_call++ & 3;
  if (!st->upd_ev[ring]) HIPCHK(hipEventCreateWithFlags(&st->upd_ev[ring], hipEventDisableTiming));
  if (st->upd_ev_set[(ring + 2) & 3]) HIPCHK(hipEventSynchronize(st->upd_ev[(ring + 2) & 3]));
  int* list = reinterpret_cast<int*>(st->h_upd + (size_t)st->maxkf * 32) + (size_t)ring * st->maxkf;
  for (int i = 0; i < n; ++i) {
    const int slot = slots[i];
    const int par = (st->upd_par[(size_t)slot] ^= 1);
    float* u = st->h_upd + 16 * (2 * (size_t)slot + par);
    std::memcpy(u, Rcw + 9 * (size_t)i, 36); std::memcpy(u + 9, tcw + 3 * (size_t)i, 12); std::memcpy(u + 12, Ow + 3 * (size_t)i, 12);
    CmsTriKF& d = st->h_kf[(size_t)slot];
    std::memcpy(d.Rcw, Rcw + 9 * (size_t)i, 36); std::memcpy(d.tcw, tcw + 3 * (size_t)i, 12); std::memcpy(d.Ow, Ow + 3 * (size_t)i, 12);
    list[i] = slot | (par << 30);
    st->busy[(size_t)slot] = 1;
  }
  hipLaunchKernelGGL(k_kf_update_poses, dim3((n + 63) / 64), dim3(64), 0, c->stream, st->d_kf, (const float*)st->h_upd, (const int*)list, n);
  HIPCHK(hipGetLastError());
  HIPCHK(hipEventRecord(st->upd_ev[ring], c->stream));
  st->upd_ev_set[ring] = true;
  return CMS_OK;
}

extern "C" int cms_kfstore_debug_fetch(cms_kfstore* st, int slot, cms_keypoint* kps, uint8_t* desc, float* rays, int* mp, int* feat_node, uint16_t* sorted,
                                       int* node_id, int* node_off, int* node_feat, int* cell_start, uint32_t* header, int* misc) {
  if (!st || slot < 0 || slot >= st->maxkf || !st->used[(size_t)slot]) return cms_fail(CMS_ERR_ARG, "cms_kfstore_debug_fetch: bad slot");
  cms_ctx* c = st->c;
  HIPCHK(hipSetDevice(c->device));
  HIPCHK(kfstore_order_behind_puts(st));
  HIPCHK(hipStreamSynchronize(c->stream));
  CmsTriKF d;
  HIPCHK(hipMemcpy(&d, st->d_kf + slot, sizeof(d), hipMemcpyDeviceToHost));
  static_assert(sizeof(CmsTriKF) == 21 * 4, "CmsTriKF is 21 words");
  if (header) std::memcpy(header, &d, sizeof(d));
  const size_t f0 = (size_t)slot * st->maxf, n0 = (size_t)slot * st->maxn, o0 = (size_t)slot * (st->maxn + 1);
  const size_t n = (size_t)std::max(0, std::min(d.n, st->maxf)), nn = (size_t)std::max(0, std::min(d.nnodes, st->maxn));
  auto dl = [&](void* dst, const void* src, size_t bytes) { return (!dst || bytes == 0) ? hipSuccess : hipMemcpy(dst, src, bytes, hipMemcpyDeviceToHost); };
  HIPCHK(dl(kps, st->d_kp + f0, n * sizeof(CmsKeyPoint))); HIPCHK(dl(desc, st->d_desc + 32 * f0, 32 * n)); HIPCHK(dl(rays, st->d_rays + 3 * f0, 12 * n));
  HIPCHK(dl(mp, st->d_mp + f0, 4 * n)); HIPCHK(dl(feat_node, st->d_fn + f0, 4 * n)); HIPCHK(dl(sorted, st->d_sorted + f0, 2 * n));
  HIPCHK(dl(node_id, st->d_nid + n0, 4 * nn)); HIPCHK(dl(node_off, st->d_noff + o0, 4 * (nn + 1)));
  int nfeat = 0;
  if (nn > 0) HIPCHK(hipMemcpy(&nfeat, st->d_noff + o0 + nn, 4, hipMemcpyDeviceToHost));
  HIPCHK(dl(node_feat, st->d_nfeat + f0, 4 * (size_t)std::max(0, std::min(nfeat, st->maxf))));
  HIPCHK(dl(cell_start, st->d_cell_start + (size_t)slot * (CMS_AREA_CELLS + 1), 4 * ((size_t)CMS_AREA_CELLS + 1)));
  if (misc) { HIPCHK(hipMemcpy(misc, st->d_nvalid + slot, 4, hipMemcpyDeviceToHost)); HIPCHK(hipMemcpy(misc + 1, st->d_kp_cnt + slot, 4, hipMemcpyDeviceToHost)); }
  return CMS_OK;
}

extern "C" int cms_kfstore_update(cms_kfstore* st, int slot, const float* Rcw, const float* tcw, const float* Ow, const float* median_depth, const int* mp) {
  if (!st || slot < 0 || slot >= st->maxkf || !st->used[(size_t)slot]) return cms_fail(CMS_ERR_ARG, "cms_kfstore_update: bad slot");
  cms_ctx* c = st->c;
  HIPCHK(hipSetDevice(c->device));
  HIPCHK(kfstore_order_behind_puts(st));
  CmsTriKF& d = st->h_kf[(size_t)slot];
  if (Rcw) std::memcpy(d.Rcw, Rcw, sizeof(d.Rcw));
  if (tcw) std::memcpy(d.tcw, tcw, sizeof(d.tcw));
  if (Ow) std::memcpy(d.Ow, Ow, sizeof(d.Ow));
  if (median_depth) st->h_median[(size_t)slot] = *median_depth;
  if (Rcw || tcw || Ow) HIPCHK(hipMemcpyAsync(st->d_kf + slot, &d, sizeof(d), hipMemcpyHostToDevice, c->stream));
  if (mp && d.n > 0) HIPCHK(hipMemcpyAsync(st->d_mp + (size_t)d.f0, mp, 4 * (size_t)d.n, hipMemcpyHostToDevice, c->stream));
  HIPCHK(hipStreamSynchronize(c->stream));
  return CMS_OK;
}

extern "C" int cms_kfstore_create_new_map_points(cms_kfstore* st, int njobs, const int* cur_slot, const int* neigh_off, const int* neigh_slot,
                                                 int check_orientation, int cap_per_job, int* n_new, int* out_neigh, int* out_idx1, int* out_idx2,
                                                 float* out_x3d) {
  if (!st || njobs < 0 || cap_per_job < 0 || (njobs > 0 && (!cur_slot || !neigh_off || !n_new)) ||
      (njobs > 0 && cap_per_job > 0 && (!out_neigh || !out_idx1 || !out_idx2 || !out_x3d)))
    return cms_fail(CMS_ERR_ARG, "cms_kfstore_create_new_map_points: bad argument");
  if (njobs == 0) return CMS_OK;
  cms_ctx* c = st->c;
  if (c->g.nlevels > 16 || c->g.nlevels < 2) return cms_fail(CMS_ERR_UNSUPPORTED, "cms_kfstore_create_new_map_points: 2..16 pyramid levels");
  const int nneigh = neigh_off[njobs];
  if (nneigh < 0 || (nneigh > 0 && !neigh_slot)) return cms_fail(CMS_ERR_ARG, "cms_kfstore_create_new_map_points: bad neighbour list");
  for (int j = 0; j < njobs; ++j)
    if (cur_slot[j] < 0 || cur_slot[j] >= st->maxkf || !st->used[(size_t)cur_slot[j]]) return cms_fail(CMS_ERR_ARG, "cms_kfstore_create_new_map_points: empty slot");
  for (int q = 0; q < nneigh; ++q)
    if (neigh_slot[q] < 0 || neigh_slot[q] >= st->maxkf || !st->used[(size_t)neigh_slot[q]]) return cms_fail(CMS_ERR_ARG, "cms_kfstore_create_new_map_points: empty slot");
  HIPCHK(hipSetDevice(c->device));
  HIPCHK(kfstore_order_behind_puts(st));
  const size_t need = TriWork(njobs, nneigh, st->maxf, cap_per_job).bytes;
  if (need > st->work_bytes) {
    if (st->d_work) HIPCHK(hipFree(st->d_work));
    st->d_work = nullptr; st->work_bytes = 0;
    HIPCHK(hipMalloc((void**)&st->d_work, need + need / 4));
    st->work_bytes = need + need / 4;
  }
  TriDev dev;
  dev.kf = st->d_kf; dev.kp = st->d_kp; dev.desc = (const uint4*)st->d_desc; dev.rays = st->d_rays; dev.mp = st->d_mp; dev.feat_node = st->d_fn;
  dev.node_id = st->d_nid; dev.node_off = st->d_noff; dev.node_feat = st->d_nfeat;
  return tri_run(c, dev, st->h_kf.data(), st->h_median.data(), njobs, cur_slot, neigh_off, neigh_slot, check_orientation, cap_per_job, st->d_work, n_new,
                 out_neigh, out_idx1, out_idx2, out_x3d);
}

static CmsFuseArgs fuse_project_args(const cms_ctx* c, int n, float th, const void* pose15, const void* mp_frame, const void* skip, const void* src, const void* P,
                                     const void* normal, const void* min_dist, const void* max_dist, const CmsWindowCols& w) {
  CmsFuseArgs a = {};
  a.pose15 = (const float*)pose15; a.mp_frame = (const int*)mp_frame; a.n = n; a.skip = (const uint8_t*)skip; a.src = (const int*)src;
  a.P = (const float*)P; a.normal = (const float*)normal; a.min_dist = (const float*)min_dist; a.max_dist = (const float*)max_dist;
  a.th = th; a.log_scale = std::log(c->scale[1]); a.nlevels = c->g.nlevels; a.F = c->g.F; a.bounds_scaled = c->dist_bounds_scaled;
  cms_level_table(a.sf, c, c->scale, 0.0f);
  a.qx = w.qx; a.qy = w.qy; a.qr = w.qr; a.qmin = w.qmin; a.qmax = w.qmax; a.level = w.level;
  return a;
}
static CmsWindowScanArgs cms_window_scan_args(const cms_ctx* g, int n, const CmsWindowCols& w, int cap, const int* src, const void* mp_desc, const CmsKeyPoint* kp,
                                              const void* t_desc, const int* row_slot, int maxf, int* best_idx, int* best_dist) {
  CmsWindowScanArgs a = {};
  a.n = n; a.qx = w.qx; a.qy = w.qy; a.level = w.level; a.src = src; a.mp_desc = (const uint4*)mp_desc;
  a.cand_off = w.off; a.cand_idx = w.idx; a.cap = cap; a.kp = kp; a.t_desc = (const uint4*)t_desc;
  cms_level_table(a.inv_sigma2, g, g->inv_sigma2, 0.0f);
  a.row_slot = row_slot; a.maxf = maxf; a.best_idx = best_idx; a.best_dist = best_dist;
  return a;
}
static unsigned cms_window_scan_grid(int n) { return (unsigned)(((size_t)n * 8 + 255) / 256); }
static int kfstore_window_query(const cms_kfstore* st, cms_ctx* ctx, hipStream_t s, const CmsWindowCols& w, int E, int cap, void* d_total) {
  CmsAreaArgs a = cms_area_args(st->d_kp, st->d_sorted, st->d_cell_start, st->maxf, st->c->g.F, cms_grid_inv(st->c));
  cms_area_queries(a, E, w, cap);
  return cms_area_launch(ctx, s, a, d_total);
}

extern "C" int cms_fuse_search(cms_ctx* c, int b, const float* pose15, int nmp, const uint8_t* skip, const float* pos, const float* normal,
                               const float* min_dist, const float* max_dist, const uint8_t* mp_desc, float th, int* best_idx, int* best_dist) {
  if (!c || !pose15 || nmp < 0 || (nmp > 0 && (!pos || !normal || !min_dist || !max_dist || !mp_desc || !best_idx || !best_dist)))
    return cms_fail(CMS_ERR_ARG, "cms_fuse_search: bad argument");
  if (b < 0 || b >= c->area_frames) return cms_fail(CMS_ERR_ARG, "cms_fuse_search: no grid for this key frame (cms_area_grid first)");
  if (nmp == 0) return CMS_OK;
  if (c->g.nlevels > 16) return cms_fail(CMS_ERR_UNSUPPORTED, "cms_fuse_search: more than 16 pyramid levels");
  HIPCHK(hipSetDevice(c->device));
  hipStream_t s = c->stream;
  const size_t n4 = (size_t)nmp * 4;
  CmsBlock blk;
  CmsWindowCols w;
  const size_t o_pose = blk.take(64), o_skip = blk.take(nmp), o_pos = blk.take(3 * n4), o_nrm = blk.take(3 * n4), o_min = blk.take(n4), o_max = blk.take(n4),
               o_desc = blk.take((size_t)nmp * 32), o_tot = blk.take(16), o_bi = blk.take(n4), o_bd = blk.take(n4);
  w.take(blk, (size_t)nmp);
  const size_t o_idx = blk.size;
  return cms_retry_capacity(64 * nmp + 1024, "cms_fuse_search", [&](int cap, int& tot) -> int {
    int rc = c->stage.reserve(s, o_idx + cms_align((size_t)cap * 4), 0);
    if (rc) return rc;
    uint8_t* p = c->stage.d;
    w.at(p, o_idx);
    HIPCHK(hipMemcpyAsync(p + o_pose, pose15, 60, hipMemcpyHostToDevice, s));
    if (skip) HIPCHK(hipMemcpyAsync(p + o_skip, skip, nmp, hipMemcpyHostToDevice, s));
    HIPCHK(hipMemcpyAsync(p + o_pos, pos, 3 * n4, hipMemcpyHostToDevice, s));
    HIPCHK(hipMemcpyAsync(p + o_nrm, normal, 3 * n4, hipMemcpyHostToDevice, s));
    HIPCHK(hipMemcpyAsync(p + o_min, min_dist, n4, hipMemcpyHostToDevice, s));
    HIPCHK(hipMemcpyAsync(p + o_max, max_dist, n4, hipMemcpyHostToDevice, s));
    HIPCHK(hipMemcpyAsync(p + o_desc, mp_desc, (size_t)nmp * 32, hipMemcpyHostToDevice, s));
    const std::vector<int> qf((size_t)nmp, b);
    HIPCHK(hipMemcpyAsync(w.slot, qf.data(), n4, hipMemcpyHostToDevice, s));
    const CmsFuseArgs fa = fuse_project_args(c, nmp, th, p + o_pose, nullptr, skip ? p + o_skip : nullptr, nullptr, p + o_pos, p + o_nrm, p + o_min, p + o_max, w);
    hipLaunchKernelGGL(k_fuse_project, dim3((nmp + 255) / 256), dim3(256), 0, s, fa);
    HIPCHK(hipGetLastError());
    rc = cms_features_in_area_batch_device(c, nmp, w.slot, w.qx, w.qy, w.qr, w.qmin, w.qmax, w.cnt, w.off, w.idx, cap, p + o_tot);
    if (rc) return rc;
    HIPCHK(hipMemcpyAsync(&tot, p + o_tot, sizeof(int), hipMemcpyDeviceToHost, s));
    HIPCHK(hipStreamSynchronize(s));
    if (tot > cap) return CMS_OK;
    const CmsWindowScanArgs sa = cms_window_scan_args(c, nmp, w, cap, nullptr, p + o_desc, (const CmsKeyPoint*)c->d_kps, c->d_desc, nullptr, 0, (int*)(p + o_bi), (int*)(p + o_bd));
    hipLaunchKernelGGL(k_fuse_scan, dim3(cms_window_scan_grid(nmp)), dim3(256), 0, s, sa);
    HIPCHK(hipGetLastError());
    HIPCHK(hipMemcpyAsync(best_idx, p + o_bi, n4, hipMemcpyDeviceToHost, s));
    HIPCHK(hipMemcpyAsync(best_dist, p + o_bd, n4, hipMemcpyDeviceToHost, s));
    HIPCHK(hipStreamSynchronize(s));
    const int base = b * c->g.kp_cap;
    for (int i = 0; i < nmp; ++i) if (best_idx[i] >= 0) best_idx[i] -= base;
    return CMS_OK;
  });
}

extern "C" int cms_distinctive_descriptors(cms_ctx* c, int npts, const int* obs_off, const uint8_t* desc, int* best_idx) {
  if (!c || npts < 0 || (npts > 0 && (!obs_off || !best_idx))) return cms_fail(CMS_ERR_ARG, "cms_distinctive_descriptors: bad argument");
  if (npts == 0) return CMS_OK;
  const int nobs = obs_off[npts];
  if (nobs < 0 || (nobs > 0 && !desc)) return cms_fail(CMS_ERR_ARG, "cms_distinctive_descriptors: bad observation list");
  for (int p = 0; p < npts; ++p) {
    if (obs_off[p + 1] < obs_off[p]) return cms_fail(CMS_ERR_ARG, "cms_distinctive_descriptors: obs_off must ascend");
    if (obs_off[p + 1] - obs_off[p] > 65535) return cms_fail(CMS_ERR_UNSUPPORTED, "cms_distinctive_descriptors: more than 65535 observations of one point");
  }
  HIPCHK(hipSetDevice(c->device));
  CmsBlock blk;
  const size_t o_off = blk.take((size_t)(npts + 1) * 4), o_desc = blk.take((size_t)nobs * 32, 32), o_out = blk.take((size_t)npts * 4);
  hipStream_t s = c->stream;
  int rc = c->stage.reserve(s, blk.size, 0);
  if (rc) return rc;
  uint8_t* p = c->stage.d;
  HIPCHK(hipMemcpyAsync(p + o_off, obs_off, (size_t)(npts + 1) * 4, hipMemcpyHostToDevice, s));
  if (nobs > 0) HIPCHK(hipMemcpyAsync(p + o_desc, desc, (size_t)nobs * 32, hipMemcpyHostToDevice, s));
  hipLaunchKernelGGL(k_distinctive, dim3((npts + 3) / 4), dim3(256), 0, s, npts, (const int*)(p + o_off), (const uint4*)(p + o_desc), (int*)(p + o_out));
  HIPCHK(hipGetLastError());
  HIPCHK(hipMemcpyAsync(best_idx, p + o_out, (size_t)npts * 4, hipMemcpyDeviceToHost, s));
  HIPCHK(hipStreamSynchronize(s));
  return CMS_OK;
}

extern "C" int cms_update_normal_and_depth(cms_ctx* c, int npts, const int* obs_off, const float* pos, const float* obs_Ow, const float* ref_Ow,
                                           const int* ref_level, float* normal, float* min_dist, float* max_dist) {
  if (!c || npts < 0 || (npts > 0 && (!obs_off || !pos || !ref_Ow || !ref_level || !normal || !min_dist || !max_dist)))
    return cms_fail(CMS_ERR_ARG, "cms_update_normal_and_depth: bad argument");
// ... 152 lines not shown
```

cubemapslam_amd/csrc/cms_area_kernels.hip:

```cpp
#include <hip/hip_runtime.h>
#include <stdint.h>
#include "cms_types.h"
#include "cms_area_table.h"
#include "cms_area_offsets.h"

#define CMS_AREA_CELLS (5 * CMS_AREA_G * CMS_AREA_G)
#define CMS_AREA_MAXKP 16383

extern "C" __global__ void __launch_bounds__(1024)
k_area_grid(const CmsKeyPoint* __restrict__ kps, const int* __restrict__ kp_cnt, int kp_cap, int F, float inv,
            uint16_t* __restrict__ sorted_idx, int* __restrict__ cell_start, int* __restrict__ n_valid_out) {
  extern __shared__ uint32_t area_lds[];
  uint32_t* keys = area_lds;
  uint32_t* sorted = area_lds + (kp_cap + 1);
  __shared__ int s_nvalid;
  const int b = blockIdx.x, tid = threadIdx.x, T = blockDim.x;
  const int n = min(kp_cnt[b], min(kp_cap, CMS_AREA_MAXKP));
  const CmsKeyPoint* kp = kps + (size_t)b * kp_cap;
  if (tid == 0) s_nvalid = 0;
  __syncthreads();
  for (int i = tid; i < n; i += T) {
    const float x = kp[i].x, y = kp[i].y;
    const double fi = (double)(x / (float)F), fj = (double)(y / (float)F);
    int f = -1;
    if (fi >= 0 && fi < 1 && fj >= 1 && fj < 2) f = 1;
    else if (fi >= 1 && fi < 2 && fj >= 0 && fj < 1) f = 3;
    else if (fi >= 1 && fi < 2 && fj >= 1 && fj < 2) f = 0;
    else if (fi >= 1 && fi < 2 && fj >= 2 && fj < 3) f = 4;
    else if (fi >= 2 && fi < 3 && fj >= 1 && fj < 2) f = 2;
    uint32_t key = 0xFFFFC000u | (uint32_t)i;
    if (f >= 0) {
      const int px = (int)(x * inv) % CMS_AREA_G, py = (int)(y * inv) % CMS_AREA_G;
      key = ((uint32_t)((f * CMS_AREA_G + px) * CMS_AREA_G + py) << 14) | (uint32_t)i;
      atomicAdd(&s_nvalid, 1);
    }
    keys[i] = key;
  }
  __syncthreads();
  for (int i = tid; i < n; i += T) {
    const uint32_t k = keys[i];
    int r = 0;
    for (int q = 0; q < n; ++q) r += keys[q] < k ? 1 : 0;
    sorted[r] = k;
  }
  __syncthreads();
  const int nv = s_nvalid;
  uint16_t* si = sorted_idx + (size_t)b * kp_cap;
  int* cs = cell_start + (size_t)b * (CMS_AREA_CELLS + 1);
  for (int s = tid; s < nv; s += T) {
    const int c = (int)(sorted[s] >> 14), prev = s ? (int)(sorted[s - 1] >> 14) : -1;
    si[s] = (uint16_t)(sorted[s] & 0x3FFFu);
    for (int cc = prev + 1; cc <= c; ++cc) cs[cc] = s;
  }
  const int last = nv ? (int)(sorted[nv - 1] >> 14) : -1;
  for (int cc = last + 1 + tid; cc <= CMS_AREA_CELLS; cc += T) cs[cc] = nv;
  if (tid == 0) n_valid_out[b] = nv;
}

struct CmsAreaArgs {
  const CmsKeyPoint* kp;
  const uint16_t* sorted_idx;
  const int* cell_start;
  const float* qx; const float* qy; const float* qr; const int* qmin; const int* qmax;
  const int* q_frame;
  int kp_cap;
  int nq, F; float inv;
  int* cnt;
  int* off;
  int* idx; int cap; int idx_base;
  int* tmp;
  int* psum;
};
#define CMS_AREA_TMP 8

__device__ __forceinline__ int cms_area_pick(int k, int v0, int v1, int v2) { return k == 0 ? v0 : (k == 1 ? v1 : v2); }

template <bool FILL>
__device__ __forceinline__ int cms_area_search(const CmsAreaArgs& a, int qq, bool in, int gl, int base) {
  const float x = a.qx[qq], y = a.qy[qq], r = a.qr[qq];
  const bool live = in && !(r < 0.0f);
  const int minLevel = a.qmin[qq], maxLevel = a.qmax[qq];
  const bool check = (minLevel > 0) || (maxLevel >= 0);
  CmsAreaRectI rc[3] = {};
  const int nr = live ? cms_area_rects(x, y, r, a.F, a.inv, rc) : 0;
  int n = 0;
  int* tmpq = a.tmp + (size_t)qq * CMS_AREA_TMP;
  const int fr = a.q_frame ? a.q_frame[qq] : 0;
  const CmsKeyPoint* kp = a.kp + (size_t)fr * a.kp_cap;
  const uint16_t* sorted_idx = a.sorted_idx + (size_t)fr * a.kp_cap;
  const int* cell_start = a.cell_start + (size_t)fr * (CMS_AREA_CELLS + 1);
  const int idx_base = a.idx_base + (a.q_frame ? fr * a.kp_cap : 0);
  for (int k = 0; k < 3; ++k) {
    const bool has = k < nr;
    const int x0 = has ? max(0, cms_area_pick(k, rc[0].x0, rc[1].x0, rc[2].x0)) : 0, x1 = has ? min(CMS_AREA_G - 1, cms_area_pick(k, rc[0].x1, rc[1].x1, rc[2].x1)) : -1;
    const int y0 = has ? max(0, cms_area_pick(k, rc[0].y0, rc[1].y0, rc[2].y0)) : 0, y1 = has ? min(CMS_AREA_G - 1, cms_area_pick(k, rc[0].y1, rc[1].y1, rc[2].y1)) : -1;
    const int face = has ? cms_area_pick(k, rc[0].face, rc[1].face, rc[2].face) : 0;
    const int ncol = (x1 >= x0 && y1 >= y0) ? x1 - x0 + 1 : 0;
    int maxcol = ncol;
    for (int o = 32; o > 0; o >>= 1) maxcol = max(maxcol, __shfl_xor(maxcol, o));
    for (int cb = 0; cb < maxcol; cb += CMS_AREA_QL) {
      const int ix = x0 + cb + gl;
      const bool col = cb + gl < ncol;
      int s0 = 0, s1 = 0;
      if (col) {
        const int c0 = (face * CMS_AREA_G + ix) * CMS_AREA_G + y0;
        s0 = cell_start[c0]; s1 = cell_start[c0 + (y1 - y0) + 1];
      }
      int h0 = 0, h1 = 0, h2 = 0, h3 = 0;
      int nh = 0;
      for (int s = s0; s < s1; ++s) {
        const int j = sorted_idx[s];
        const CmsKeyPoint p = kp[j];
        if (check) {
          if (p.octave < minLevel) continue;
          if (maxLevel >= 0 && p.octave > maxLevel) continue;
        }
        if (fabsf(p.x - x) < r && fabsf(p.y - y) < r) {
          if (nh == 0) h0 = j; else if (nh == 1) h1 = j; else if (nh == 2) h2 = j; else if (nh == 3) h3 = j;
          ++nh;
        }
      }
      int incl = nh;
#pragma unroll
      for (int o = 1; o < CMS_AREA_QL; o <<= 1) { const int t = __shfl_up(incl, o, CMS_AREA_QL); if (gl >= o) incl += t; }
      const int tot = __shfl(incl, CMS_AREA_QL - 1, CMS_AREA_QL);
      if (!FILL && nh > 0) {
        int w = n + incl - nh;
        if (w < CMS_AREA_TMP) {
          if (nh <= 4) {
            tmpq[w] = idx_base + h0;
            if (nh > 1 && w + 1 < CMS_AREA_TMP) tmpq[w + 1] = idx_base + h1;
            if (nh > 2 && w + 2 < CMS_AREA_TMP) tmpq[w + 2] = idx_base + h2;
            if (nh > 3 && w + 3 < CMS_AREA_TMP) tmpq[w + 3] = idx_base + h3;
          } else {
            for (int s = s0; s < s1 && w < CMS_AREA_TMP; ++s) {
              const int j = sorted_idx[s];
              const CmsKeyPoint p = kp[j];
              if (check && (p.octave < minLevel || (maxLevel >= 0 && p.octave > maxLevel))) continue;
              if (fabsf(p.x - x) < r && fabsf(p.y - y) < r) { tmpq[w] = idx_base + j; ++w; }
            }
          }
        }
      }
      if (FILL && nh > 0) {
        int w = base + n + incl - nh;
        if (nh <= 4) {
          if (cms_area_fits(w, a.cap)) a.idx[w] = idx_base + h0;
          if (nh > 1 && cms_area_fits(w + 1, a.cap)) a.idx[w + 1] = idx_base + h1;
          if (nh > 2 && cms_area_fits(w + 2, a.cap)) a.idx[w + 2] = idx_base + h2;
          if (nh > 3 && cms_area_fits(w + 3, a.cap)) a.idx[w + 3] = idx_base + h3;
        } else {
          for (int s = s0; s < s1; ++s) {
            const int j = sorted_idx[s];
            const CmsKeyPoint p = kp[j];
            if (check && (p.octave < minLevel || (maxLevel >= 0 && p.octave > maxLevel))) continue;
            if (fabsf(p.x - x) < r && fabsf(p.y - y) < r) { if (cms_area_fits(w, a.cap)) a.idx[w] = idx_base + j; ++w; }
          }
        }
      }
      n += tot;
    }
  }
  return n;
}

extern "C" __global__ void __launch_bounds__(CMS_AREA_QT) k_area_query(CmsAreaArgs a) {
  __shared__ int part[CMS_AREA_QT / 64];
  const int gl = threadIdx.x & (CMS_AREA_QL - 1);
  const int q = (blockIdx.x * CMS_AREA_QT + threadIdx.x) / CMS_AREA_QL;
  const bool in = q < a.nq;
  const int n = cms_area_search<false>(a, in ? q : 0, in, gl, 0);
  if (in && gl == 0) a.cnt[q] = n;
  int v = n;
  for (int o = CMS_AREA_QL; o < 64; o <<= 1) v += __shfl_xor(v, o);
  if ((threadIdx.x & 63) == 0) part[threadIdx.x >> 6] = v;
  __syncthreads();
  if (threadIdx.x == 0) { int t = 0; for (int w = 0; w < CMS_AREA_QT / 64; ++w) t += part[w]; a.psum[blockIdx.x] = t; }
}

extern "C" __global__ void __launch_bounds__(CMS_AREA_LT) k_area_lists(CmsAreaArgs a, int* __restrict__ total) {
  __shared__ int s_cnt[CMS_AREA_TILE], s_off[CMS_AREA_TILE];
  __shared__ int part[CMS_AREA_TILE_K * CMS_AREA_LW], pbefore[CMS_AREA_LW];
  const int tid = threadIdx.x, lane = tid & 63, wv = tid >> 6;
  const int tile = blockIdx.x, q0 = tile * CMS_AREA_TILE;
  int before = 0;
  {
    const int4* p4 = (const int4*)a.psum;
    const int n4 = cms_area_parts_before(tile) / 4;
    for (int b = tid; b < n4; b += CMS_AREA_LT) { const int4 v = p4[b]; before += (v.x + v.y) + (v.z + v.w); }
  }
  for (int o = 32; o > 0; o >>= 1) before += __shfl_xor(before, o);
  if (lane == 0) pbefore[wv] = before;
  int c[CMS_AREA_TILE_K], incl[CMS_AREA_TILE_K];
#pragma unroll
  for (int k = 0; k < CMS_AREA_TILE_K; ++k) {
    const int q = q0 + cms_area_tile_slot(tid, k);
    c[k] = q < a.nq ? a.cnt[q] : 0;
    int s = c[k];
#pragma unroll
    for (int o = 1; o < 64; o <<= 1) { const int t = __shfl_up(s, o); if (lane >= o) s += t; }
    incl[k] = s;
    if (lane == 63) part[k * CMS_AREA_LW + wv] = s;
  }
  __syncthreads();
  int tile_base = 0;
  for (int w = 0; w < CMS_AREA_LW; ++w) tile_base += pbefore[w];
#pragma unroll
  for (int k = 0; k < CMS_AREA_TILE_K; ++k) {
    const int ql = cms_area_tile_slot(tid, k), q = q0 + ql;
    const int mine = tile_base + cms_area_handover(part, k, wv) + incl[k];
    s_cnt[ql] = c[k]; s_off[ql] = mine - c[k];
    if (q < a.nq) a.off[q + 1] = mine;
    if (q == a.nq - 1 && total) *total = mine;
  }
  if (tile == 0 && tid == 0) a.off[0] = 0;
  __syncthreads();
  const int gl = tid & (CMS_AREA_QL - 1), g = tid / CMS_AREA_QL;
  const int nt = min(CMS_AREA_TILE, a.nq - q0);
  for (int t0 = 0; t0 < nt; t0 += 4 * CMS_AREA_LG) {
    int v[4], w[4]; bool ok[4];
#pragma unroll
    for (int u = 0; u < 4; ++u) {
      const int ql = t0 + u * CMS_AREA_LG + g;
      const bool in = ql < nt;
      const int cq = in ? s_cnt[ql] : 0;
      w[u] = (in ? s_off[ql] : 0) + gl;
      ok[u] = cq <= CMS_AREA_TMP && gl < cq && cms_area_fits(w[u], a.cap);
      v[u] = a.tmp[(size_t)(in ? q0 + ql : q0) * CMS_AREA_TMP + gl];
    }
#pragma unroll
    for (int u = 0; u < 4; ++u) if (ok[u]) a.idx[w[u]] = v[u];
  }
  for (int t0 = 0; t0 < nt; t0 += CMS_AREA_LG) {
    const int ql = t0 + g;
    const bool big = ql < nt && s_cnt[ql] > CMS_AREA_TMP;
    if (__ballot(big)) cms_area_search<true>(a, big ? q0 + ql : q0, big, gl, big ? s_off[ql] : 0);
  }
}
```

include/cubemapslam_hip.h:

```cpp
#ifndef CUBEMAPSLAM_HIP_H
#define CUBEMAPSLAM_HIP_H
#include <stddef.h>
#include <stdint.h>
#ifdef __cplusplus
extern "C" {
#endif

#define CMS_OK 0
#define CMS_ERR_ARG (-1)
#define CMS_ERR_HIP (-2)
#define CMS_ERR_UNSUPPORTED (-3)
#define CMS_ERR_OVERFLOW (-4)
#define CMS_ERR_NO_DEVICE (-5)

enum { CMS_FACE_UNKNOWN = -1, CMS_FACE_FRONT = 0, CMS_FACE_LEFT = 1, CMS_FACE_RIGHT = 2, CMS_FACE_UPPER = 3, CMS_FACE_LOWER = 4 };

typedef struct {
  double c, d, e, u0, v0;
  double invpol[12];
  double pol[5];
  int Iw, Ih;
  int face;
  double fov_deg;
} cms_camera;
// ... 44 lines not shown
int cms_frames_results(cms_ctx* ctx, void** d_kps, void** d_desc, void** d_counts);
int cms_frames_fetch(cms_ctx* ctx, int b, cms_keypoint* kps, uint8_t* desc, int cap, int* n);

typedef struct { uint16_t tx, ty, x0, y0, nd, rows, flags, pad; } cms_remap_tile;
int cms_remap_lut_host(const cms_camera* cam, uint32_t* lut, int lut_stride);
int cms_remap_tiles_host(const cms_camera* cam, const uint32_t* lut, int lut_stride, int tile_w, int tile_h, int lds_budget,
                         cms_remap_tile* out, int cap, int* n_live, int* n_all, int* lds_bytes);

int cms_fast_cells_host(const cms_camera* cam, const cms_orb_params* orb, int which, int* out, int cap, int* n);

int cms_debug_lut(cms_ctx* ctx, uint32_t* out, int* stride);
int cms_debug_cubemap(cms_ctx* ctx, int b, uint8_t* dst, int dstride);
int cms_debug_level(cms_ctx* ctx, int b, int level, uint8_t* dst, int dstride);
int cms_debug_candidates(cms_ctx* ctx, int b, int level, int* xys, int cap, int* n);
int cms_debug_distributed(cms_ctx* ctx, int b, int level, int* xys, int cap, int* n);

int cms_profile_enable(cms_ctx* ctx, int on);
int cms_profile_get(cms_ctx* ctx, float* ms7);

int cms_hamming_best2(cms_ctx* ctx, const uint8_t* qdesc, int nq, const uint8_t* tdesc, int nt, const int* cand_off,
                      const int* cand_idx, const int* t_level, const uint8_t* t_excluded, int* best_idx, int* best_dist,
                      int* best_level, int* second_dist, int* second_level);
int cms_hamming_best2_device(cms_ctx* ctx, const void* qdesc, const void* q_row, int nq, const void* tdesc, const void* cand_off,
                             const void* cand_idx, const void* t_level, const void* t_excluded, void* best_idx,
                             void* best_dist, void* best_level, void* second_dist, void* second_level);
int cms_hamming_matrix(cms_ctx* ctx, const uint8_t* a, int na, const uint8_t* b, int nb, uint16_t* out);

typedef struct cms_ba cms_ba;
typedef struct {
  int iterations_done[2];
  double chi2_initial[2], chi2_final[2], lambda_final[2];
  int n_outliers_mid, n_outliers_final;
} cms_ba_stats;
int cms_ba_create(cms_ba** out, int device, int K, const double* poses, const uint8_t* fixed, int P, const double* points,
                  int E, const int* e_pose, const int* e_point, const double* e_obs, const double* e_invsig2,
                  const int8_t* e_face, double fx, double fy, double cx, double cy);
typedef struct cms_ba_window {
  int K; const double* poses; const uint8_t* fixed; int P; const double* points; int E; const int* e_pose; const int* e_point;
  const double* e_obs; const double* e_invsig2; const int8_t* e_face; double fx, fy, cx, cy;
  int flags;
} cms_ba_window;
#define CMS_BA_INPUTS_PINNED 1
#define CMS_BA_PLAN_ON_DEVICE 2
int cms_ba_create_many(cms_ba** out, int n, int device, const cms_ba_window* windows, int threads);
int cms_ba_read_many(cms_ba** bas, int n, double** poses, double** points, uint8_t** outlier_flags);
int cms_ba_reset(cms_ba* ba);
int cms_ba_optimize(cms_ba* ba, int its_robust, int its_final, const volatile uint8_t* stop, cms_ba_stats* stats);
int cms_ba_optimize_many(cms_ba** bas, int n, int its_robust, int its_final, const volatile uint8_t* stop, cms_ba_stats* stats);
int cms_ba_optimize_global(cms_ba* ba, int iterations, int robust, const volatile uint8_t* stop, cms_ba_stats* stats);
int cms_ba_optimize_global_many(cms_ba** bas, int n, int iterations, int robust, const volatile uint8_t* stop, cms_ba_stats* stats);
int cms_ba_debug_solve_tiled(int device, int n, const double* A, const double* b, double* x, int* status);
int cms_ba_debug_solve_timed(int device, int which, int n, const double* A, const double* b, double* x, int* status, int reps, double* ms);
int cms_ba_read(cms_ba* ba, double* poses, double* points, uint8_t* outlier_flags);
void* cms_ba_stream(cms_ba* ba);
int cms_ba_set_stream(cms_ba* ba, void* hip_stream);
int cms_ba_debug_clocks(cms_ba* ba, long long* out16);
int cms_ba_profile_kernel(cms_ba* ba, int kernel_id);
int cms_ba_profile_get(cms_ba* ba, double* total_ms, long* launches);
int cms_ba_debug_compose(int K, const uint8_t* fixed, int P, int E, const int* e_pose, const int* e_point, int lookahead,
                         int* pinv, int* chunk_pt0, int* n_chunks, uint8_t* rank);
int cms_ba_debug_plan(int K, const uint8_t* fixed, int P, int E, const int* e_pose, const int* e_point, int* pinv, int* perm, uint32_t* info,
                      int* chunk_pt0, int* rm_chunk, uint32_t* run_lane, int* counts, uint32_t* run_mf, uint32_t* run_fl);
int cms_ba_debug_fetch_plan(cms_ba* ba, int* pinv, int* perm, uint32_t* info, int* pt_off, int* e_pose, int* e_point, int8_t* e_face, int* chunk_e0,
                            int* rm_chunk, uint32_t* rm_cost, uint32_t* run_mf, uint32_t* run_fl, int* counts);
int cms_ba_debug_plan_fast(int K, const uint8_t* fixed, int P, int E, const int* e_pose, const int* e_point, int* pinv, int* perm, uint32_t* info,
                           int* chunk_pt0, int* rm_chunk, int* counts, uint32_t* run_mf, uint32_t* run_fl);
int cms_ba_debug_run_fg(int K, const uint8_t* fixed, int P, int E, const int* e_pose, const int* e_point, int fast, uint32_t* run_fg, int* rm_cut, int* counts);
int cms_ba_debug_match(int which, int n, const int* slots, int np, int* choice_out);
void cms_ba_destroy(cms_ba* ba);
int cms_ba_pool_trim(int device, size_t* released);
int cms_ba_set_deterministic(int on);
int cms_ba_get_deterministic(void);
int cms_ba_run(int device, int K, double* poses, const uint8_t* fixed, int P, double* points, int E, const int* e_pose,
               const int* e_point, const double* e_obs, const double* e_invsig2, const int8_t* e_face, double fx, double fy,
               double cx, double cy, int its_robust, int its_final, const volatile uint8_t* stop, uint8_t* outlier_flags,
               cms_ba_stats* stats);
int cms_ba_linearize(int device, int K, const double* poses, const uint8_t* fixed, int P, const double* points, int E,
                     const int* e_pose, const int* e_point, const double* e_obs, const double* e_invsig2,
                     const int8_t* e_face, double fx, double fy, double cx, double cy, int robust, double huber_delta,
                     double* err, double* Hpp, double* bp, double* Hll, double* bl, double* Hpl, double* robust_chi2_sum);

int cms_area_set_keypoints(cms_ctx* ctx, int b, int n, const cms_keypoint* kps);
int cms_area_grid(cms_ctx* ctx, int B);
int cms_features_in_area(cms_ctx* ctx, int b, int nq, const float* qx, const float* qy, const float* qr, const int* min_level,
                         const int* max_level, int* cand_off, int* cand_idx, int cap, int* total);
int cms_features_in_area_device(cms_ctx* ctx, int b, int nq, const void* d_qx, const void* d_qy, const void* d_qr, const void* d_min_level,
                                const void* d_max_level, void* d_cnt_scratch, void* d_cand_off, void* d_cand_idx, int cap, int idx_base,
                                void* d_total);
int cms_features_in_area_batch_device(cms_ctx* ctx, int nq, const void* d_qframe, const void* d_qx, const void* d_qy, const void* d_qr,
                                      const void* d_min_level, const void* d_max_level, void* d_cnt_scratch, void* d_cand_off,
                                      void* d_cand_idx, int cap, void* d_total);

int cms_area_set_descriptors(cms_ctx* ctx, int b, int n, const uint8_t* desc);
int cms_set_distance_bounds_mode(cms_ctx* ctx, int scaled);
int cms_search_by_projection(cms_ctx* ctx, int b, const float* pose12, int nlast, const uint8_t* valid, const float* Xw, const int* octave,
                             const float* angle, const uint8_t* mp_desc, float th, int check_orientation, int th_high, int nkp, int* kp_mp,
                             int* match, int* n_matches);
int cms_search_for_initialization(cms_ctx* ctx, int b2, int n1, const cms_keypoint* kps1, const uint8_t* desc1, float* prev_matched,
                                  int window_size, float nnratio, int check_orientation, int* matches12, int* n_matches);
int cms_project_last_frame_device(cms_ctx* ctx, int n, const void* d_qframe, const void* d_pose12, const void* d_valid, const void* d_Xw,
                                  const void* d_oct, float th, void* d_qx, void* d_qy, void* d_qr, void* d_qmin, void* d_qmax);
int cms_rotation_filter_device(cms_ctx* ctx, int B, const void* d_mp_off, const void* d_last_angle, void* d_kp_mp, void* d_mp_match,
                               void* d_n_matches, int check_orientation);
int cms_search_local_points(cms_ctx* ctx, int b, const float* pose15, int nmp, const float* pos, const float* normal,
                            const float* min_dist, const float* max_dist, const uint8_t* mp_desc, float viewing_cos_limit, float th,
                            float nnratio, int th_high, int nkp, int* kp_mp, uint8_t* in_view, float* proj_x, float* proj_y, int* level,
                            float* view_cos, int* mp_match, int* n_matches, int* rounds);
int cms_is_in_frustum_device(cms_ctx* ctx, int nmp, const void* d_mp_frame, const void* d_pose15, const void* d_pos, const void* d_normal,
                             const void* d_min_dist, const void* d_max_dist, float viewing_cos_limit, float th, void* d_in_view,
                             void* d_proj_x, void* d_proj_y, void* d_level, void* d_view_cos, void* d_qr, void* d_qmin, void* d_qmax);
int cms_search_local_points_device(cms_ctx* ctx, int B, const void* d_mp_off, const void* d_mp_desc, const void* d_cand_off,
                                   const void* d_cand_idx, void* d_pair_dist, float nnratio, int th_high, void* d_kp_mp, void* d_mp_match,
                                   void* d_rounds);

typedef struct {
  int n; const cms_keypoint* kps; const uint8_t* desc; const float* rays; const int* mp;
  float Rcw[9], tcw[3], Ow[3];
  int nnodes; const int* node_id; const int* node_off; const int* node_feat;
  float median_depth;
} cms_keyframe;
int cms_create_new_map_points(cms_ctx* ctx, int njobs, const cms_keyframe* cur, const int* neigh_off, const cms_keyframe* neigh,
                              int check_orientation, int cap_per_job, int* n_new, int* out_neigh, int* out_idx1, int* out_idx2,
                              float* out_x3d);
int cms_search_for_triangulation(cms_ctx* ctx, const cms_keyframe* kf1, const cms_keyframe* kf2, const float* E12, int check_orientation,
                                 int* matches12, int* n_matches);
typedef struct cms_kfstore cms_kfstore;
int cms_kfstore_create(cms_kfstore** out, cms_ctx* ctx, int max_keyframes, int max_features, int max_nodes);
void cms_kfstore_destroy(cms_kfstore* st);
int cms_kfstore_put(cms_kfstore* st, int slot, const cms_keyframe* kf);
int cms_kfstore_update(cms_kfstore* st, int slot, const float* Rcw, const float* tcw, const float* Ow, const float* median_depth, const int* mp);
int cms_kfstore_put_from_frame(cms_kfstore* st, int slot, cms_ctx* src, int b, int n, const float* Rcw, const float* tcw, const float* Ow, float median_depth,
                               const int* mp, int nnodes, const int* node_id, const int* node_off, const int* node_feat);
typedef struct {
  int slot, b, n;
  const float* Rcw; const float* tcw; const float* Ow; float median_depth;
  const int* mp; int nnodes; const int* node_id; const int* node_off; const int* node_feat;
} cms_kf_from_frame;
int cms_kfstore_put_from_frames(cms_kfstore* st, cms_ctx* src, int n_items, const cms_kf_from_frame* items);
int cms_kfstore_update_poses(cms_kfstore* st, int n, const int* slots, const float* Rcw, const float* tcw, const float* Ow);
int cms_kfstore_debug_fetch(cms_kfstore* st, int slot, cms_keypoint* kps, uint8_t* desc, float* rays, int* mp, int* feat_node, uint16_t* sorted,
                            int* node_id, int* node_off, int* node_feat, int* cell_start, uint32_t* header, int* misc);
int cms_kfstore_fuse_search(cms_kfstore* st, int njobs, const int* job_slot, const int* mp_off, const uint8_t* skip, const float* pos,
                            const float* normal, const float* min_dist, const float* max_dist, const uint8_t* mp_desc, float th, int* best_idx,
                            int* best_dist);
int cms_kfstore_fuse_search_sets(cms_kfstore* st, int nsets, const int* set_off, const float* pos, const float* normal, const float* min_dist,
                                 const float* max_dist, const uint8_t* mp_desc, int njobs, const int* job_slot, const int* job_set, const uint8_t* skip,
                                 float th, int* best_idx, int* best_dist);
int cms_kfstore_create_new_map_points(cms_kfstore* st, int njobs, const int* cur_slot, const int* neigh_off, const int* neigh_slot,
                                      int check_orientation, int cap_per_job, int* n_new, int* out_neigh, int* out_idx1, int* out_idx2,
                                      float* out_x3d);
int cms_distinctive_descriptors(cms_ctx* ctx, int npts, const int* obs_off, const uint8_t* desc, int* best_idx);
int cms_update_normal_and_depth(cms_ctx* ctx, int npts, const int* obs_off, const float* pos, const float* obs_Ow, const float* ref_Ow,
                                const int* ref_level, float* normal, float* min_dist, float* max_dist);
int cms_fuse_search(cms_ctx* ctx, int b, const float* pose15, int nmp, const uint8_t* skip, const float* pos, const float* normal,
                    const float* min_dist, const float* max_dist, const uint8_t* mp_desc, float th, int* best_idx, int* best_dist);

int cms_search_by_bow(cms_ctx* ctx, int b, int n, int nnodes, const int* node_id, const int* node_off, const int* node_feat,
                      const cms_keyframe* kf, const uint8_t* kf_skip, float nnratio, int check_orientation,
                      int* kf_idx , int* n_matches);
typedef struct {
  int slot;
  int b, n;
  int nnodes; const int* node_id; const int* node_off; const int* node_feat;
  const uint8_t* kf_skip;
} cms_bow_job;
int cms_kfstore_search_by_bow(cms_kfstore* st, cms_ctx* src, int njobs, const cms_bow_job* jobs, float nnratio,
                              int check_orientation, int* kf_idx , int* n_matches );

typedef struct {
  int slot1, n1;
  int slot2, n2;
  const uint8_t* skip1;
  const uint8_t* skip2;
} cms_bow_kf_job;
int cms_kfstore_search_by_bow_keyframes(cms_kfstore* st, cms_ctx* src, int njobs, const cms_bow_kf_job* jobs,
                                        float nnratio, int check_orientation,
                                        int* idx2 , int* n_matches );

typedef struct cms_vocab cms_vocab;
int cms_vocab_create(cms_vocab** out, int device, int k, int L, int scoring, int weighting, int n_nodes, const int* parent, const uint8_t* is_leaf,
                     const uint8_t* desc, const double* weight);
void cms_vocab_destroy(cms_vocab* v);
int cms_vocab_info(const cms_vocab* v, int* info);
int cms_vocab_profile_enable(int on);
int cms_vocab_profile_get(float* ms2);
int cms_vocab_transform(cms_vocab* v, cms_ctx* ctx, int n, const uint8_t* desc, int levelsup, int* nwords, int* word_id, double* word_val, int* nnodes,
                        int* node_id, int* node_off, int* node_feat);
int cms_frames_compute_bow(cms_ctx* ctx, cms_vocab* v, int levelsup, int n_rows, const int* rows, const int* n);
int cms_frames_fetch_bow(cms_ctx* ctx, int b, int* nwords, int* word_id, double* word_val, int word_cap, int* nnodes, int* node_id, int* node_off,
                         int* node_feat, int node_cap, int feat_cap);
int cms_kfstore_compute_bow(cms_kfstore* st, cms_vocab* v, int levelsup, int n_slots, const int* slots);
int cms_kfstore_fetch_bow(cms_kfstore* st, int slot, int* nwords, int* word_id, double* word_val, int word_cap, int* nnodes, int* node_id, int* node_off,
                          int* node_feat, int node_cap, int feat_cap);
int cms_kfstore_search_by_bow_frames(cms_kfstore* st, cms_ctx* src, int njobs, const cms_bow_job* jobs, float nnratio, int check_orientation,
                                     int* kf_idx, int* n_matches);

int cms_kfstore_set_bow(cms_kfstore* st, int slot, int nwords, const int* word_id, const double* word_val);
int cms_kfdb_add(cms_kfstore* st, int n, const int* slots, const int* groups);
int cms_kfdb_erase(cms_kfstore* st, int n, const int* slots);
int cms_kfdb_clear(cms_kfstore* st, int group);
int cms_kfdb_set_covisibles(cms_kfstore* st, int n, const int* slots, const int* neigh);
#define CMS_KFDB_RELOC 0
#define CMS_KFDB_LOOP 1
#define CMS_KFDB_QUERY_ROW 0
#define CMS_KFDB_QUERY_SLOT 1
#define CMS_KFDB_QUERY_WORDS 2
typedef struct cms_kfdb_job {
  int mode, group, query;
  int b, slot;
  int nwords; const int* word_id; const double* word_val;
  float min_score; int n_connected; const int* connected;
} cms_kfdb_job;
int cms_kfdb_detect(cms_kfstore* st, cms_ctx* src, int njobs, const cms_kfdb_job* jobs, int cand_cap, int* cand_slot, int* n_cand, int* diag_common,
                    float* diag_score);
int cms_kfstore_bow_score(cms_kfstore* st, int npairs, const int* slot_a, const int* slot_b, double* score);
int cms_kfdb_profile_enable(int on);
int cms_kfdb_profile_get(float* ms);

typedef struct {
  int slot;
  int b, n;
  float pose12[12];
  int nmp;
  const int* kf_feat;
// ... 177 lines not shown
```

Before: 25530.

## Store packed per-cell keypoint records for area queries instead of indirect lookups

The grid build now also writes a packed int4 record per sorted keypoint, holding position, octave and index, so area queries read contiguous records rather than going through sorted_idx and then gathering the keypoint. The query loop is restructured to flatten columns across all rectangles into a single pass sequence and to prefetch the first four records per column. The records are copied into the keyframe store as well. This costs extra memory and extra writes and copies when grids are built, in exchange for fewer dependent gathers in the query.

Result: faster. 25900, median of 5 (+1.4%).

```diff
diff --git a/cubemapslam_amd/api.py b/cubemapslam_amd/api.py
--- a/cubemapslam_amd/api.py
+++ b/cubemapslam_amd/api.py
@@ -408,6 +408,16 @@
     def area_grid(self, B):
         _chk(lib().cms_area_grid(self.h, B), "cms_area_grid")
 
+    def area_debug_fetch(self, b):
+        cap = self.geom.kp_cap
+        o = dict(kps=np.zeros(cap, KP_DTYPE), sorted=np.zeros(cap, np.uint16), rec=np.zeros((cap, 4), np.uint32), cell_start=np.zeros(5 * 50 * 50 + 1, np.int32))
+        misc = np.zeros(2, np.int32)
+        L = lib()
+        L.cms_area_debug_fetch.argtypes = [C.c_void_p, C.c_int] + [C.c_void_p] * 5
+        _chk(L.cms_area_debug_fetch(self.h, b, _p(o["kps"]), _p(o["sorted"]), _p(o["rec"]), _p(o["cell_start"]), _p(misc)), "cms_area_debug_fetch")
+        o["nvalid"] = int(misc[0]); o["kp_cnt"] = int(misc[1])
+        return o
+
     def features_in_area(self, b, qx, qy, qr, qmin, qmax, cap=None):
         qx = np.ascontiguousarray(qx, np.float32); qy = np.ascontiguousarray(qy, np.float32); qr = np.ascontiguousarray(qr, np.float32)
         qmin = np.ascontiguousarray(qmin, np.int32); qmax = np.ascontiguousarray(qmax, np.int32)
@@ -813,6 +823,15 @@
         o["node_feat"] = o["node_feat"][:int(o["node_off"][-1]) if nn else 0]
         o["header"] = hdr; o["nvalid"] = int(misc[0]); o["kp_cnt"] = int(misc[1])
         return o
+
+    def debug_fetch_records(self, slot):
+        hdr = np.zeros(21, np.uint32); misc = np.zeros(2, np.int32)
+        L = lib()
+        _chk(L.cms_kfstore_debug_fetch(self.h, slot, *([None] * 10), _p(hdr), _p(misc)), "cms_kfstore_debug_fetch")
+        rec = np.zeros((max(int(hdr[1]), 1), 4), np.uint32)
+        L.cms_kfstore_debug_fetch_records.argtypes = [C.c_void_p, C.c_int, C.c_void_p]
+        _chk(L.cms_kfstore_debug_fetch_records(self.h, slot, _p(rec)), "cms_kfstore_debug_fetch_records")
+        return rec[:int(hdr[1])]
 
     def update_map_points(self, slot, feat, mp):
         a = [np.ascontiguousarray(v, np.int32).reshape(-1) for v in (slot, feat, mp)]
diff --git a/cubemapslam_amd/csrc/cms_api_area.hip b/cubemapslam_amd/csrc/cms_api_area.hip
--- a/cubemapslam_amd/csrc/cms_api_area.hip
+++ b/cubemapslam_amd/csrc/cms_api_area.hip
@@ -10,6 +10,7 @@
   { const int rca = cms_area_grid_attr(c->device); if (rca) return rca; }
   const size_t B = (size_t)c->max_batch;
   HIPCHK(hipMalloc((void**)&c->d_area_sorted, B * c->g.kp_cap * sizeof(uint16_t)));
+  HIPCHK(hipMalloc((void**)&c->d_area_rec, B * c->g.kp_cap * sizeof(int4)));
   HIPCHK(hipMalloc((void**)&c->d_area_cell_start, B * (CMS_AREA_CELLS + 1) * sizeof(int)));
   HIPCHK(hipMalloc((void**)&c->d_area_nvalid, B * sizeof(int)));
   return CMS_OK;
@@ -34,14 +35,13 @@
   return CMS_OK;
 }
 
-static CmsAreaArgs cms_area_args(const CmsKeyPoint* kp, const uint16_t* sorted_idx, const int* cell_start, int kp_cap, int F, float inv) {
+static CmsAreaArgs cms_area_args(const int4* rec, const int* cell_start, int kp_cap, int F, float inv) {
   CmsAreaArgs a = {};
-  a.kp = kp; a.sorted_idx = sorted_idx; a.cell_start = cell_start; a.kp_cap = kp_cap; a.F = F; a.inv = inv;
+  a.rec = rec; a.cell_start = cell_start; a.kp_cap = kp_cap; a.F = F; a.inv = inv;
   return a;
 }
 static CmsAreaArgs cms_area_args_frames(const cms_ctx* c, int b) {
-  return cms_area_args((const CmsKeyPoint*)c->d_kps + (size_t)b * c->g.kp_cap, c->d_area_sorted + (size_t)b * c->g.kp_cap,
-                       c->d_area_cell_start + (size_t)b * (CMS_AREA_CELLS + 1), c->g.kp_cap, c->g.F, cms_grid_inv(c));
+  return cms_area_args(c->d_area_rec + (size_t)b * c->g.kp_cap, c->d_area_cell_start + (size_t)b * (CMS_AREA_CELLS + 1), c->g.kp_cap, c->g.F, cms_grid_inv(c));
 }
 static void cms_area_queries(CmsAreaArgs& a, int nq, const void* q_frame, const void* qx, const void* qy, const void* qr, const void* qmin, const void* qmax,
                              void* cnt, void* off, void* idx, int cap, int idx_base) {
@@ -95,9 +95,21 @@
   int rc = cms_area_reserve(c);
   if (rc) return rc;
   hipLaunchKernelGGL(k_area_grid, dim3(B), dim3(1024), (size_t)(c->g.kp_cap + 1) * 8, c->stream, (const CmsKeyPoint*)c->d_kps, (const int*)c->d_kp_cnt, c->g.kp_cap, c->g.F, cms_grid_inv(c),
-                     c->d_area_sorted, c->d_area_cell_start, c->d_area_nvalid);
+                     c->d_area_sorted, c->d_area_rec, c->d_area_cell_start, c->d_area_nvalid);
   HIPCHK(hipGetLastError());
   c->area_frames = B;
+  return CMS_OK;
+}
+
+extern "C" int cms_area_debug_fetch(cms_ctx* c, int b, cms_keypoint* kps, uint16_t* sorted, uint32_t* rec, int* cell_start, int* misc) {
+  if (!c || b < 0 || b >= c->area_frames) return cms_fail(CMS_ERR_ARG, "cms_area_debug_fetch: no grid for this frame (cms_area_grid first)");
+  HIPCHK(hipSetDevice(c->device));
+  HIPCHK(hipStreamSynchronize(c->stream));
+  const size_t cap = (size_t)c->g.kp_cap, f0 = (size_t)b * cap;
+  auto dl = [&](void* dst, const void* src, size_t bytes) { return !dst ? hipSuccess : hipMemcpy(dst, src, bytes, hipMemcpyDeviceToHost); };
+  HIPCHK(dl(kps, c->d_kps + f0, cap * sizeof(cms_keypoint))); HIPCHK(dl(sorted, c->d_area_sorted + f0, cap * sizeof(uint16_t)));
+  HIPCHK(dl(rec, c->d_area_rec + f0, cap * sizeof(int4))); HIPCHK(dl(cell_start, c->d_area_cell_start + (size_t)b * (CMS_AREA_CELLS + 1), 4 * ((size_t)CMS_AREA_CELLS + 1)));
+  if (misc) { HIPCHK(hipMemcpy(misc, c->d_area_nvalid + b, 4, hipMemcpyDeviceToHost)); HIPCHK(hipMemcpy(misc + 1, c->d_kp_cnt + b, 4, hipMemcpyDeviceToHost)); }
   return CMS_OK;
 }
 
diff --git a/cubemapslam_amd/csrc/cms_api_frames.hip b/cubemapslam_amd/csrc/cms_api_frames.hip
--- a/cubemapslam_amd/csrc/cms_api_frames.hip
+++ b/cubemapslam_amd/csrc/cms_api_frames.hip
@@ -76,7 +76,7 @@
   uint32_t* d_qt_out = nullptr; int* d_qt_cnt = nullptr;
   uint32_t* d_cell_cand = nullptr; int* d_cell_cnt = nullptr;
   int* d_cells_all = nullptr; int* d_cells_live = nullptr; int n_cells_all = 0, n_cells_live = 0;
-  uint16_t* d_area_sorted = nullptr; int* d_area_cell_start = nullptr; int* d_area_nvalid = nullptr; int area_frames = 0;
+  uint16_t* d_area_sorted = nullptr; int4* d_area_rec = nullptr; int* d_area_cell_start = nullptr; int* d_area_nvalid = nullptr; int area_frames = 0;
   int* d_area_psum = nullptr; int area_psum_cap = 0;
   int* d_area_tmp = nullptr; size_t area_tmp_cap = 0;
   uint8_t* h_fish_stage = nullptr; int fish_stage_frames = 0;
@@ -353,7 +353,7 @@
   hipSetDevice(c->device);
   void* ptrs[] = {c->d_fish, c->d_lut, c->d_pyr, c->d_mask, c->d_tab, c->d_pattern, c->d_cand, c->d_node, c->d_cand_cnt,
                   c->d_overflow, c->d_qt_out, c->d_qt_cnt, c->d_kps, c->d_aux, c->d_order, c->d_aux_sorted, c->d_desc, c->d_kp_cnt, c->d_cell_cand,
-                  c->d_cell_cnt, c->d_cells_all, c->d_cells_live, c->d_area_sorted, c->d_area_cell_start, c->d_area_nvalid, c->d_area_psum, c->d_area_tmp, c->d_walk_cnt, c->d_rays, c->d_rtiles};
+                  c->d_cell_cnt, c->d_cells_all, c->d_cells_live, c->d_area_sorted, c->d_area_rec, c->d_area_cell_start, c->d_area_nvalid, c->d_area_psum, c->d_area_tmp, c->d_walk_cnt, c->d_rays, c->d_rtiles};
   for (void* p : ptrs) if (p) hipFree(p);
   cms_ctx_bow_free(c->bow);
   if (c->h_fish_stage) (void)hipHostFree(c->h_fish_stage);
diff --git a/cubemapslam_amd/csrc/cms_api_tri.hip b/cubemapslam_amd/csrc/cms_api_tri.hip
--- a/cubemapslam_amd/csrc/cms_api_tri.hip
+++ b/cubemapslam_amd/csrc/cms_api_tri.hip
@@ -312,7 +312,7 @@
   CmsTriKF* d_kf = nullptr; CmsKeyPoint* d_kp = nullptr; uint8_t* d_desc = nullptr; float* d_rays = nullptr; int* d_mp = nullptr; int* d_fn = nullptr;
   int* d_nid = nullptr; int* d_noff = nullptr; int* d_nfeat = nullptr;
   uint8_t* d_work = nullptr; size_t work_bytes = 0;
-  uint16_t* d_sorted = nullptr; int* d_cell_start = nullptr; int* d_nvalid = nullptr; int* d_kp_cnt = nullptr;
+  uint16_t* d_sorted = nullptr; int4* d_rec = nullptr; int* d_cell_start = nullptr; int* d_nvalid = nullptr; int* d_kp_cnt = nullptr;
   std::vector<CmsTriKF> h_kf; std::vector<float> h_median; std::vector<uint8_t> used;
   struct PutCall { hipEvent_t ev = nullptr; ~PutCall() { if (ev) (void)hipEventDestroy(ev); } };
   int* h_ff = nullptr; size_t ff_stride = 0; std::vector<std::shared_ptr<PutCall>> ff_call;
@@ -336,7 +336,7 @@
   if (!st) return;
   if (st->c) (void)hipSetDevice(st->c->device);
   void* bufs[] = {st->d_kf, st->d_kp, st->d_desc, st->d_rays, st->d_mp, st->d_fn, st->d_nid, st->d_noff, st->d_nfeat, st->d_work,
-                  st->d_sorted, st->d_cell_start, st->d_nvalid, st->d_kp_cnt};
+                  st->d_sorted, st->d_rec, st->d_cell_start, st->d_nvalid, st->d_kp_cnt};
   for (void* b : bufs) if (b) (void)hipFree(b);
   cms_store_bow_free(st->bow);
   cms_store_kfdb_free(st->kfdb);
@@ -368,6 +368,7 @@
   KF_ALLOC(st->d_noff, K * (Nq + 1) * 4);
   KF_ALLOC(st->d_nfeat, K * Fq * 4);
   KF_ALLOC(st->d_sorted, K * Fq * sizeof(uint16_t));
+  KF_ALLOC(st->d_rec, K * Fq * sizeof(int4));
   KF_ALLOC(st->d_cell_start, K * (CMS_AREA_CELLS + 1) * sizeof(int));
   KF_ALLOC(st->d_nvalid, K * sizeof(int));
   KF_ALLOC(st->d_kp_cnt, K * sizeof(int));
@@ -413,7 +414,7 @@
   HIPCHK(hipMemcpyAsync(st->d_kf + slot, &d, sizeof(d), hipMemcpyHostToDevice, s));
   HIPCHK(hipMemcpyAsync(st->d_kp_cnt + slot, &kf->n, sizeof(int), hipMemcpyHostToDevice, s));
   hipLaunchKernelGGL(k_area_grid, dim3(1), dim3(1024), (size_t)(st->maxf + 1) * 8, s, (const CmsKeyPoint*)(st->d_kp + f0), (const int*)(st->d_kp_cnt + slot), st->maxf, c->g.F,
-                     cms_grid_inv(c), st->d_sorted + f0, st->d_cell_start + (size_t)slot * (CMS_AREA_CELLS + 1), st->d_nvalid + slot);
+                     cms_grid_inv(c), st->d_sorted + f0, st->d_rec + f0, st->d_cell_start + (size_t)slot * (CMS_AREA_CELLS + 1), st->d_nvalid + slot);
   HIPCHK(hipGetLastError());
   HIPCHK(hipStreamSynchronize(s));
   st->h_kf[(size_t)slot] = d; st->h_median[(size_t)slot] = kf->median_depth; st->used[(size_t)slot] = 1;
@@ -423,8 +424,8 @@
 }
 
 struct CmsKfFromFrame {
-  const CmsKeyPoint* kp; const uint8_t* desc; const float* rays; const uint16_t* sorted; const int* cell_start; const int* nvalid;
-  CmsKeyPoint* o_kp; uint8_t* o_desc; float* o_rays; uint16_t* o_sorted; int* o_cell_start; int* o_nvalid; int* o_kp_cnt;
+  const CmsKeyPoint* kp; const uint8_t* desc; const float* rays; const uint16_t* sorted; const int4* rec; const int* cell_start; const int* nvalid;
+  CmsKeyPoint* o_kp; uint8_t* o_desc; float* o_rays; uint16_t* o_sorted; int4* o_rec; int* o_cell_start; int* o_nvalid; int* o_kp_cnt;
   int* o_mp; int* o_fn; int* o_nid; int* o_noff; int* o_nfeat; CmsTriKF* o_kf;
   const int* h_mp; const int* h_fn; const int* h_nid; const int* h_noff; const int* h_nfeat;
   CmsTriKF kf; int n, nnodes, nfeat;
@@ -442,6 +443,7 @@
     for (int i = t0; i < 2 * n; i += gs) d[i] = s[i];
   }
   for (int i = t0; i < 3 * n; i += gs) a.o_rays[i] = a.rays[i];
+  for (int i = t0; i < n; i += gs) a.o_rec[i] = a.rec[i];
   for (int i = t0; i < n; i += gs) { a.o_sorted[i] = a.sorted[i]; a.o_mp[i] = a.h_mp ? a.h_mp[i] : -1; a.o_fn[i] = a.h_fn[i]; }
   for (int i = t0; i <= CMS_AREA_CELLS; i += gs) a.o_cell_start[i] = a.cell_start[i];
   for (int i = t0; i < a.nnodes; i += gs) a.o_nid[i] = a.h_nid[i];
@@ -504,9 +506,9 @@
   d.f0 = (int)f0; d.n = n; d.node0 = (int)n0; d.nnodes = nnodes; d.noff0 = (int)o0; d.nfeat0 = (int)f0;
   std::memcpy(d.Rcw, Rcw, sizeof(d.Rcw)); std::memcpy(d.tcw, tcw, sizeof(d.tcw)); std::memcpy(d.Ow, Ow, sizeof(d.Ow));
   const size_t sb = (size_t)b * src->g.kp_cap;
-  a.kp = (const CmsKeyPoint*)src->d_kps + sb; a.desc = src->d_desc + 32 * sb; a.rays = src->d_rays + 3 * sb; a.sorted = src->d_area_sorted + sb;
+  a.kp = (const CmsKeyPoint*)src->d_kps + sb; a.desc = src->d_desc + 32 * sb; a.rays = src->d_rays + 3 * sb; a.sorted = src->d_area_sorted + sb; a.rec = src->d_area_rec + sb;
   a.cell_start = src->d_area_cell_start + (size_t)b * (CMS_AREA_CELLS + 1); a.nvalid = src->d_area_nvalid + b;
-  a.o_kp = st->d_kp + f0; a.o_desc = st->d_desc + 32 * f0; a.o_rays = st->d_rays + 3 * f0; a.o_sorted = st->d_sorted + f0;
+  a.o_kp = st->d_kp + f0; a.o_desc = st->d_desc + 32 * f0; a.o_rays = st->d_rays + 3 * f0; a.o_sorted = st->d_sorted + f0; a.o_rec = st->d_rec + f0;
   a.o_cell_start = st->d_cell_start + (size_t)slot * (CMS_AREA_CELLS + 1); a.o_nvalid = st->d_nvalid + slot; a.o_kp_cnt = st->d_kp_cnt + slot;
   a.o_mp = st->d_mp + f0; a.o_fn = st->d_fn + f0; a.o_nid = st->d_nid + n0; a.o_noff = st->d_noff + o0; a.o_nfeat = st->d_nfeat + f0; a.o_kf = st->d_kf + slot;
   a.h_mp = mp ? h_mp : nullptr; a.h_fn = h_fn; a.h_nid = h_nid; a.h_noff = h_noff; a.h_nfeat = h_nfeat;
@@ -641,6 +643,17 @@
   return CMS_OK;
 }
 
+extern "C" int cms_kfstore_debug_fetch_records(cms_kfstore* st, int slot, uint32_t* rec) {
+  if (!st || !rec || slot < 0 || slot >= st->maxkf || !st->used[(size_t)slot]) return cms_fail(CMS_ERR_ARG, "cms_kfstore_debug_fetch_records: bad slot");
+  cms_ctx* c = st->c;
+  HIPCHK(hipSetDevice(c->device));
+  HIPCHK(kfstore_order_behind_puts(st));
+  HIPCHK(hipStreamSynchronize(c->stream));
+  const size_t n = (size_t)std::max(0, std::min(st->h_kf[(size_t)slot].n, st->maxf));
+  if (n > 0) HIPCHK(hipMemcpy(rec, st->d_rec + (size_t)slot * st->maxf, n * sizeof(int4), hipMemcpyDeviceToHost));
+  return CMS_OK;
+}
+
 extern "C" int cms_kfstore_update(cms_kfstore* st, int slot, const float* Rcw, const float* tcw, const float* Ow, const float* median_depth, const int* mp) {
   if (!st || slot < 0 || slot >= st->maxkf || !st->used[(size_t)slot]) return cms_fail(CMS_ERR_ARG, "cms_kfstore_update: bad slot");
   cms_ctx* c = st->c;
@@ -709,7 +722,7 @@
 }
 static unsigned cms_window_scan_grid(int n) { return (unsigned)(((size_t)n * 8 + 255) / 256); }
 static int kfstore_window_query(const cms_kfstore* st, cms_ctx* ctx, hipStream_t s, const CmsWindowCols& w, int E, int cap, void* d_total) {
-  CmsAreaArgs a = cms_area_args(st->d_kp, st->d_sorted, st->d_cell_start, st->maxf, st->c->g.F, cms_grid_inv(st->c));
+  CmsAreaArgs a = cms_area_args(st->d_rec, st->d_cell_start, st->maxf, st->c->g.F, cms_grid_inv(st->c));
   cms_area_queries(a, E, w, cap);
   return cms_area_launch(ctx, s, a, d_total);
 }
diff --git a/cubemapslam_amd/csrc/cms_area_columns.h b/cubemapslam_amd/csrc/cms_area_columns.h
--- /dev/null
+++ b/cubemapslam_amd/csrc/cms_area_columns.h
@@ -0,0 +1,41 @@
+#ifndef CMS_AREA_COLUMNS_H
+#define CMS_AREA_COLUMNS_H
+#include "cms_area_table.h"
+#include "cms_area_offsets.h"
+
+struct CmsAreaCols {
+  CmsAreaRectI r0, r1, r2;
+  int n0, n1, n2;
+};
+struct CmsAreaCol { int face, ix, y0, y1; };
+
+AREA_FN CmsAreaRectI cms_area_clamp(const CmsAreaRectI& r, bool has) {
+  CmsAreaRectI c;
+  c.face = has ? r.face : 0;
+  c.x0 = has ? (r.x0 < 0 ? 0 : r.x0) : 0; c.x1 = has ? (r.x1 > CMS_AREA_G - 1 ? CMS_AREA_G - 1 : r.x1) : -1;
+  c.y0 = has ? (r.y0 < 0 ? 0 : r.y0) : 0; c.y1 = has ? (r.y1 > CMS_AREA_G - 1 ? CMS_AREA_G - 1 : r.y1) : -1;
+  return c;
+}
+AREA_FN int cms_area_ncol(const CmsAreaRectI& c) { return (c.x1 >= c.x0 && c.y1 >= c.y0) ? c.x1 - c.x0 + 1 : 0; }
+
+AREA_FN CmsAreaCols cms_area_cols(const CmsAreaRectI& a, const CmsAreaRectI& b, const CmsAreaRectI& c, int nr) {
+  CmsAreaCols k;
+  k.r0 = cms_area_clamp(a, nr > 0); k.r1 = cms_area_clamp(b, nr > 1); k.r2 = cms_area_clamp(c, nr > 2);
+  k.n0 = cms_area_ncol(k.r0); k.n1 = cms_area_ncol(k.r1); k.n2 = cms_area_ncol(k.r2);
+  return k;
+}
+AREA_FN int cms_area_cols_total(const CmsAreaCols& k) { return k.n0 + k.n1 + k.n2; }
+AREA_FN int cms_area_passes(int total) { return (total + CMS_AREA_QL - 1) / CMS_AREA_QL; }
+AREA_FN int cms_area_lane_column(int p, int gl) { return p * CMS_AREA_QL + gl; }
+AREA_FN int cms_area_pick(int w, int v0, int v1, int v2) { return w == 0 ? v0 : (w == 1 ? v1 : v2); }
+AREA_FN CmsAreaCol cms_area_column(const CmsAreaCols& k, int c) {
+  const int w = c < k.n0 ? 0 : (c < k.n0 + k.n1 ? 1 : 2);
+  CmsAreaCol o;
+  o.face = cms_area_pick(w, k.r0.face, k.r1.face, k.r2.face);
+  o.ix = cms_area_pick(w, k.r0.x0, k.r1.x0, k.r2.x0) + (c - cms_area_pick(w, 0, k.n0, k.n0 + k.n1));
+  o.y0 = cms_area_pick(w, k.r0.y0, k.r1.y0, k.r2.y0);
+  o.y1 = cms_area_pick(w, k.r0.y1, k.r1.y1, k.r2.y1);
+  return o;
+}
+
+#endif
diff --git a/cubemapslam_amd/csrc/cms_area_kernels.hip b/cubemapslam_amd/csrc/cms_area_kernels.hip
--- a/cubemapslam_amd/csrc/cms_area_kernels.hip
+++ b/cubemapslam_amd/csrc/cms_area_kernels.hip
@@ -3,13 +3,14 @@
 #include "cms_types.h"
 #include "cms_area_table.h"
 #include "cms_area_offsets.h"
+#include "cms_area_columns.h"
 
 #define CMS_AREA_CELLS (5 * CMS_AREA_G * CMS_AREA_G)
 #define CMS_AREA_MAXKP 16383
 
 extern "C" __global__ void __launch_bounds__(1024)
 k_area_grid(const CmsKeyPoint* __restrict__ kps, const int* __restrict__ kp_cnt, int kp_cap, int F, float inv,
-            uint16_t* __restrict__ sorted_idx, int* __restrict__ cell_start, int* __restrict__ n_valid_out) {
+            uint16_t* __restrict__ sorted_idx, int4* __restrict__ rec, int* __restrict__ cell_start, int* __restrict__ n_valid_out) {
   extern __shared__ uint32_t area_lds[];
   uint32_t* keys = area_lds;
   uint32_t* sorted = area_lds + (kp_cap + 1);
@@ -46,10 +47,14 @@
   __syncthreads();
   const int nv = s_nvalid;
   uint16_t* si = sorted_idx + (size_t)b * kp_cap;
+  int4* rc = rec + (size_t)b * kp_cap;
   int* cs = cell_start + (size_t)b * (CMS_AREA_CELLS + 1);
   for (int s = tid; s < nv; s += T) {
     const int c = (int)(sorted[s] >> 14), prev = s ? (int)(sorted[s - 1] >> 14) : -1;
-    si[s] = (uint16_t)(sorted[s] & 0x3FFFu);
+    const uint32_t i = sorted[s] & 0x3FFFu;
+    si[s] = (uint16_t)i;
+    const uint32_t* p = reinterpret_cast<const uint32_t*>(kp + i);
+    rc[s] = make_int4((int)p[0], (int)p[1], (int)((p[5] << 16) | i), 0);
     for (int cc = prev + 1; cc <= c; ++cc) cs[cc] = s;
   }
   const int last = nv ? (int)(sorted[nv - 1] >> 14) : -1;
@@ -58,8 +63,7 @@
 }
 
 struct CmsAreaArgs {
-  const CmsKeyPoint* kp;
-  const uint16_t* sorted_idx;
+  const int4* rec;
   const int* cell_start;
   const float* qx; const float* qy; const float* qr; const int* qmin; const int* qmax;
   const int* q_frame;
@@ -73,7 +77,10 @@
 };
 #define CMS_AREA_TMP 8
 
-__device__ __forceinline__ int cms_area_pick(int k, int v0, int v1, int v2) { return k == 0 ? v0 : (k == 1 ? v1 : v2); }
+__device__ __forceinline__ float cms_area_rec_x(const int4& v) { return __int_as_float(v.x); }
+__device__ __forceinline__ float cms_area_rec_y(const int4& v) { return __int_as_float(v.y); }
+__device__ __forceinline__ int cms_area_rec_octave(const int4& v) { return v.z >> 16; }
+__device__ __forceinline__ int cms_area_rec_index(const int4& v) { return v.z & 0xFFFF; }
 
 template <bool FILL>
 __device__ __forceinline__ int cms_area_search(const CmsAreaArgs& a, int qq, bool in, int gl, int base) {
@@ -83,83 +90,88 @@
   const bool check = (minLevel > 0) || (maxLevel >= 0);
   CmsAreaRectI rc[3] = {};
   const int nr = live ? cms_area_rects(x, y, r, a.F, a.inv, rc) : 0;
+  const CmsAreaCols cols = cms_area_cols(rc[0], rc[1], rc[2], nr);
+  const int ncol = cms_area_cols_total(cols);
   int n = 0;
   int* tmpq = a.tmp + (size_t)qq * CMS_AREA_TMP;
   const int fr = a.q_frame ? a.q_frame[qq] : 0;
-  const CmsKeyPoint* kp = a.kp + (size_t)fr * a.kp_cap;
-  const uint16_t* sorted_idx = a.sorted_idx + (size_t)fr * a.kp_cap;
+  const int4* rec = a.rec + (size_t)fr * a.kp_cap;
   const int* cell_start = a.cell_start + (size_t)fr * (CMS_AREA_CELLS + 1);
   const int idx_base = a.idx_base + (a.q_frame ? fr * a.kp_cap : 0);
-  for (int k = 0; k < 3; ++k) {
-    const bool has = k < nr;
-    const int x0 = has ? max(0, cms_area_pick(k, rc[0].x0, rc[1].x0, rc[2].x0)) : 0, x1 = has ? min(CMS_AREA_G - 1, cms_area_pick(k, rc[0].x1, rc[1].x1, rc[2].x1)) : -1;
-    const int y0 = has ? max(0, cms_area_pick(k, rc[0].y0, rc[1].y0, rc[2].y0)) : 0, y1 = has ? min(CMS_AREA_G - 1, cms_area_pick(k, rc[0].y1, rc[1].y1, rc[2].y1)) : -1;
-    const int face = has ? cms_area_pick(k, rc[0].face, rc[1].face, rc[2].face) : 0;
-    const int ncol = (x1 >= x0 && y1 >= y0) ? x1 - x0 + 1 : 0;
-    int maxcol = ncol;
-    for (int o = 32; o > 0; o >>= 1) maxcol = max(maxcol, __shfl_xor(maxcol, o));
-    for (int cb = 0; cb < maxcol; cb += CMS_AREA_QL) {
-      const int ix = x0 + cb + gl;
-      const bool col = cb + gl < ncol;
-      int s0 = 0, s1 = 0;
-      if (col) {
-        const int c0 = (face * CMS_AREA_G + ix) * CMS_AREA_G + y0;
-        s0 = cell_start[c0]; s1 = cell_start[c0 + (y1 - y0) + 1];
+  auto hit = [&](const int4& p) -> bool {
+    if (check) {
+      const int o = cms_area_rec_octave(p);
+      if (o < minLevel) return false;
+      if (maxLevel >= 0 && o > maxLevel) return false;
+    }
+    return fabsf(cms_area_rec_x(p) - x) < r && fabsf(cms_area_rec_y(p) - y) < r;
+  };
+  int passes = cms_area_passes(ncol);
+  for (int o = 32; o > 0; o >>= 1) passes = max(passes, __shfl_xor(passes, o));
+  for (int p = 0; p < passes; ++p) {
+    const int c = cms_area_lane_column(p, gl);
+    int s0 = 0, s1 = 0;
+    if (c < ncol) {
+      const CmsAreaCol cc = cms_area_column(cols, c);
+      const int c0 = (cc.face * CMS_AREA_G + cc.ix) * CMS_AREA_G + cc.y0;
+      s0 = cell_start[c0]; s1 = cell_start[c0 + (cc.y1 - cc.y0) + 1];
+    }
+    int h0 = 0, h1 = 0, h2 = 0, h3 = 0;
+    int nh = 0;
+    {
+      int4 p0 = {}, p1 = {}, p2 = {}, p3 = {};
+      if (s0 < s1) p0 = rec[s0];
+      if (s0 + 1 < s1) p1 = rec[s0 + 1];
+      if (s0 + 2 < s1) p2 = rec[s0 + 2];
+      if (s0 + 3 < s1) p3 = rec[s0 + 3];
+      if (s0 < s1 && hit(p0)) { h0 = cms_area_rec_index(p0); nh = 1; }
+      if (s0 + 1 < s1 && hit(p1)) { const int j = cms_area_rec_index(p1); if (nh == 0) h0 = j; else h1 = j; ++nh; }
+      if (s0 + 2 < s1 && hit(p2)) { const int j = cms_area_rec_index(p2); if (nh == 0) h0 = j; else if (nh == 1) h1 = j; else h2 = j; ++nh; }
+      if (s0 + 3 < s1 && hit(p3)) { const int j = cms_area_rec_index(p3); if (nh == 0) h0 = j; else if (nh == 1) h1 = j; else if (nh == 2) h2 = j; else h3 = j; ++nh; }
+    }
+    for (int s = s0 + 4; s < s1; ++s) {
+      const int4 q = rec[s];
+      if (hit(q)) {
+        const int j = cms_area_rec_index(q);
+        if (nh == 0) h0 = j; else if (nh == 1) h1 = j; else if (nh == 2) h2 = j; else if (nh == 3) h3 = j;
+        ++nh;
       }
-      int h0 = 0, h1 = 0, h2 = 0, h3 = 0;
-      int nh = 0;
-      for (int s = s0; s < s1; ++s) {
-        const int j = sorted_idx[s];
-        const CmsKeyPoint p = kp[j];
-        if (check) {
-          if (p.octave < minLevel) continue;
-          if (maxLevel >= 0 && p.octave > maxLevel) continue;
-        }
-        if (fabsf(p.x - x) < r && fabsf(p.y - y) < r) {
-          if (nh == 0) h0 = j; else if (nh == 1) h1 = j; else if (nh == 2) h2 = j; else if (nh == 3) h3 = j;
-          ++nh;
-        }
-      }
-      int incl = nh;
-#pragma unroll
-      for (int o = 1; o < CMS_AREA_QL; o <<= 1) { const int t = __shfl_up(incl, o, CMS_AREA_QL); if (gl >= o) incl += t; }
-      const int tot = __shfl(incl, CMS_AREA_QL - 1, CMS_AREA_QL);
-      if (!FILL && nh > 0) {
-        int w = n + incl - nh;
-        if (w < CMS_AREA_TMP) {
-          if (nh <= 4) {
-            tmpq[w] = idx_base + h0;
-            if (nh > 1 && w + 1 < CMS_AREA_TMP) tmpq[w + 1] = idx_base + h1;
-            if (nh > 2 && w + 2 < CMS_AREA_TMP) tmpq[w + 2] = idx_base + h2;
-            if (nh > 3 && w + 3 < CMS_AREA_TMP) tmpq[w + 3] = idx_base + h3;
-          } else {
-            for (int s = s0; s < s1 && w < CMS_AREA_TMP; ++s) {
-              const int j = sorted_idx[s];
-              const CmsKeyPoint p = kp[j];
-              if (check && (p.octave < minLevel || (maxLevel >= 0 && p.octave > maxLevel))) continue;
-              if (fabsf(p.x - x) < r && fabsf(p.y - y) < r) { tmpq[w] = idx_base + j; ++w; }
-            }
+    }
+    int incl = nh;
+#pragma unroll
+    for (int o = 1; o < CMS_AREA_QL; o <<= 1) { const int t = __shfl_up(incl, o, CMS_AREA_QL); if (gl >= o) incl += t; }
+    const int tot = __shfl(incl, CMS_AREA_QL - 1, CMS_AREA_QL);
+    if (!FILL && nh > 0) {
+      int w = n + incl - nh;
+      if (w < CMS_AREA_TMP) {
+        if (nh <= 4) {
+          tmpq[w] = idx_base + h0;
+          if (nh > 1 && w + 1 < CMS_AREA_TMP) tmpq[w + 1] = idx_base + h1;
+          if (nh > 2 && w + 2 < CMS_AREA_TMP) tmpq[w + 2] = idx_base + h2;
+          if (nh > 3 && w + 3 < CMS_AREA_TMP) tmpq[w + 3] = idx_base + h3;
+        } else {
+          for (int s = s0; s < s1 && w < CMS_AREA_TMP; ++s) {
+            const int4 q = rec[s];
+            if (hit(q)) { tmpq[w] = idx_base + cms_area_rec_index(q); ++w; }
           }
         }
       }
-      if (FILL && nh > 0) {
-        int w = base + n + incl - nh;
-        if (nh <= 4) {
-          if (cms_area_fits(w, a.cap)) a.idx[w] = idx_base + h0;
-          if (nh > 1 && cms_area_fits(w + 1, a.cap)) a.idx[w + 1] = idx_base + h1;
-          if (nh > 2 && cms_area_fits(w + 2, a.cap)) a.idx[w + 2] = idx_base + h2;
-          if (nh > 3 && cms_area_fits(w + 3, a.cap)) a.idx[w + 3] = idx_base + h3;
-        } else {
-          for (int s = s0; s < s1; ++s) {
-            const int j = sorted_idx[s];
-            const CmsKeyPoint p = kp[j];
-            if (check && (p.octave < minLevel || (maxLevel >= 0 && p.octave > maxLevel))) continue;
-            if (fabsf(p.x - x) < r && fabsf(p.y - y) < r) { if (cms_area_fits(w, a.cap)) a.idx[w] = idx_base + j; ++w; }
-          }
+    }
+    if (FILL && nh > 0) {
+      int w = base + n + incl - nh;
+      if (nh <= 4) {
+        if (cms_area_fits(w, a.cap)) a.idx[w] = idx_base + h0;
+        if (nh > 1 && cms_area_fits(w + 1, a.cap)) a.idx[w + 1] = idx_base + h1;
+        if (nh > 2 && cms_area_fits(w + 2, a.cap)) a.idx[w + 2] = idx_base + h2;
+        if (nh > 3 && cms_area_fits(w + 3, a.cap)) a.idx[w + 3] = idx_base + h3;
+      } else {
+        for (int s = s0; s < s1; ++s) {
+          const int4 q = rec[s];
+          if (hit(q)) { if (cms_area_fits(w, a.cap)) a.idx[w] = idx_base + cms_area_rec_index(q); ++w; }
         }
       }
-      n += tot;
-    }
+    }
+    n += tot;
   }
   return n;
 }
diff --git a/include/cubemapslam_hip.h b/include/cubemapslam_hip.h
--- a/include/cubemapslam_hip.h
+++ b/include/cubemapslam_hip.h
@@ -150,6 +150,7 @@
 
 int cms_area_set_keypoints(cms_ctx* ctx, int b, int n, const cms_keypoint* kps);
 int cms_area_grid(cms_ctx* ctx, int B);
+int cms_area_debug_fetch(cms_ctx* ctx, int b, cms_keypoint* kps, uint16_t* sorted, uint32_t* rec, int* cell_start, int* misc);
 int cms_features_in_area(cms_ctx* ctx, int b, int nq, const float* qx, const float* qy, const float* qr, const int* min_level,
                          const int* max_level, int* cand_off, int* cand_idx, int cap, int* total);
 int cms_features_in_area_device(cms_ctx* ctx, int b, int nq, const void* d_qx, const void* d_qy, const void* d_qr, const void* d_min_level,
@@ -208,6 +209,7 @@
 int cms_kfstore_update_poses(cms_kfstore* st, int n, const int* slots, const float* Rcw, const float* tcw, const float* Ow);
 int cms_kfstore_debug_fetch(cms_kfstore* st, int slot, cms_keypoint* kps, uint8_t* desc, float* rays, int* mp, int* feat_node, uint16_t* sorted,
                             int* node_id, int* node_off, int* node_feat, int* cell_start, uint32_t* header, int* misc);
+int cms_kfstore_debug_fetch_records(cms_kfstore* st, int slot, uint32_t* rec);
 int cms_kfstore_fuse_search(cms_kfstore* st, int njobs, const int* job_slot, const int* mp_off, const uint8_t* skip, const float* pos,
                             const float* normal, const float* min_dist, const float* max_dist, const uint8_t* mp_desc, float th, int* best_idx,
                             int* best_dist);
```
